# theEricMa/ScaleDreamer

Measured on AMD Instinct MI355X. Metric: ASD train steps/sec (64x64 render, SD2.1), higher is better.
Workload: dtype f32 renderer / f16 diffusion (f32 accumulate); 1 GPU; asd_sd_nerf: 1 view/GPU, 64x64 rays, 512 spp occgrid march, implicit-volume iNGP (16x2 hash grid 2^19, MLP 64), SD-2.1 UNet batch 5 (CFG+Perp-Neg+shifted t), VAE 512^2 fwd+bwd, AdamW; views_per_gpu=1, parallelism=dp1, diffusion_backend=hip, diffusion_weights=seeded random init (seed 1)

## Files before the change

### include/asd_hip.h

```cpp
#ifndef ASD_HIP_H
#define ASD_HIP_H

#include <stdint.h>

#ifdef __cplusplus
extern "C" {
#endif

#define ASD_MAX_LEVELS 16
#define ASD_OK 0
#define ASD_ERR_ARG 1
#define ASD_ERR_LAUNCH 2
#define ASD_ERR_UNSUPPORTED 3

typedef struct asd_grid_meta {
    uint32_t n_levels;
    uint32_t n_features;
    uint32_t n_params;
    uint32_t reserved;
    float    scale[ASD_MAX_LEVELS];
    uint32_t resolution[ASD_MAX_LEVELS];
    uint32_t offset[ASD_MAX_LEVELS];
    uint32_t size[ASD_MAX_LEVELS];
    uint32_t dense[ASD_MAX_LEVELS];
// ... 184 lines not shown
                      float* weights , float* opacity, float* depth, float* rgb_fg ,
                      float* z_var, float* comp_rgb , void* stream);
int asd_composite_bwd(int32_t mode, const float* sigma, const float* t_start, const float* t_end,
                      const float* rgb, const int32_t* offset, const int32_t* count, int32_t n_rays,
                      const float* bg, const float* weights, const float* opacity, const float* depth,
                      const float* d_comp_rgb, const float* d_rgb_fg, const float* d_opacity,
                      const float* d_depth, const float* d_z_var, const float* d_weights,
                      float* d_sigma, float* d_rgb, float* d_bg, void* stream);

typedef struct asd_render_params {
    asd_march_cfg march;
    const asd_grid_meta* meta;
    const asd_field_cfg* field;
    const float* rays_o; const float* rays_d; int32_t n_rays;
    const uint32_t* occ_bits;
    const float* jitter;
    const float* grid; const float* w1d; const float* w2d; const float* w1f; const float* w2f;
    const float* bg;
    float early_stop_eps, alpha_thre;
    int32_t prune;
    int32_t color_act;
    int32_t capacity;
} asd_render_params;
typedef struct asd_render_layout {
    int64_t total_bytes;
    int64_t count, offset, total;
    int64_t c_ray_idx, c_t0, c_t1, c_pts, c_sigma, keep;
    int64_t kept, koff, n_kept;
    int64_t ray_idx , t0, t1, pts, dirs, sigma, feats , enc, weights;
    int64_t opacity, depth, z_var, rgb_fg, comp_rgb;
    int64_t c_feats, c_enc;
} asd_render_layout;
int asd_render_layout_init(int32_t n_rays, int32_t capacity, asd_render_layout* layout);
int asd_render_fwd(const asd_render_params* p, void* workspace, void* stream);
int asd_render_bwd_workspace(const asd_render_params* p, int64_t* n_floats);
int asd_render_bwd(const asd_render_params* p, void* workspace, const float* d_comp_rgb, const float* d_rgb_fg, const float* d_opacity,
                   const float* d_depth, const float* d_z_var, float* d_grid, float* dw1d, float* dw2d, float* dw1f, float* dw2f,
                   float* d_bg, float* bwd_workspace, void* stream);

typedef struct asd_gemm_args {
    const void* A;
    const void* W;
    void*       C;
    int32_t M, N, K;
    int32_t lda, ldw, ldc;
    const void* bias;
    const void* row_bias;
    int32_t rows_per_group;
    const void* residual;
    int32_t ldr;
    int32_t act;
    int32_t out_f32;
    int32_t conv;
    int32_t Hin, Win, Cin, Hout, Wout, stride, pad;
    int32_t upsample;
    const void* zero_page;
    int32_t split_k;
    float*  workspace;
    int32_t tile_cfg;
    int32_t ld_row_bias;
    int32_t group_m, group_n;
    float*  gn_partials;
    int32_t gn_cg;
    int32_t gn_rows;
    const void* gn_bwd_x;
    const float* gn_bwd_fstats;
    const void* gn_bwd_gamma; const void* gn_bwd_beta;
    float   gn_eps;
    int32_t gn_silu;
    int32_t wide_rows;
    int32_t ln_mode;
    float   ln_eps;
    const float* ln_sc;
    float*  ln_stats;
    int32_t a_seg_rows, w_seg_rows;
    int32_t a_seg_off[9], w_seg_off[6];
    int32_t partials_only;
    int32_t gn_apply;
    void*   gn_apply_y;
    const void* gn_apply_gamma; const void* gn_apply_beta;
    float   gn_apply_eps;
    int32_t gn_apply_silu;
    float*  gn_apply_stats;
} asd_gemm_args;
int32_t asd_gemm_gn_records(const asd_gemm_args* args);
int32_t asd_gemm_gn_applies(const asd_gemm_args* args);
int asd_gemm_f16(const asd_gemm_args* args, void* stream);
int asd_gemm_force_tile(int32_t cfg);
enum { ASD_TILE_PLAIN = 0, ASD_TILE_WIN = 1, ASD_TILE_WIN2 = 2, ASD_TILE_PP = 3, ASD_TILE_WS = 4 };
int asd_gemm_tile_info(int32_t i, int32_t* out7);

#define ASD_GN_STATS_FLOATS(batch) (64 * (batch) + 64 * (512 + (batch)))
int asd_groupnorm_f16(const void* x1, int32_t c1, const void* x2, int32_t c2, int32_t batch, int32_t hw,
                      const void* gamma, const void* beta, float eps, int32_t silu, void* y,
                      float* stats ,
                      void* stream);
int asd_groupnorm_ordered_f16(const void* x, int32_t c, int32_t batch, int32_t hw, const void* gamma, const void* beta, float eps,
                              int32_t silu, void* y, float* stats, void* stream);
int asd_groupnorm_apply_f16(const void* x, int32_t c, int32_t batch, int32_t hw, const void* gamma, const void* beta, float eps,
                            int32_t silu, const float* partials, int32_t records, void* y, float* stats, void* stream);
int asd_groupnorm_bwd_f16(const void* x, const void* dy, int32_t c, int32_t batch, int32_t hw, const void* gamma,
                          const void* beta, float eps, int32_t silu, const float* fwd_stats,
                          const void* dx_add ,
                          void* dx, float* bwd_stats , void* stream);
int asd_groupnorm_bwd_apply_f16(const void* x, const void* dy, int32_t c, int32_t batch, int32_t hw, const void* gamma, const void* beta,
                                float eps, int32_t silu, const float* fwd_stats, const float* partials, int32_t records,
                                const void* dx_add, void* dx, float* scratch , void* stream);
int asd_transpose_f16(const void* x, int32_t rows, int32_t cols, int32_t ldx, void* y, int32_t ldy, void* stream);
int asd_layernorm_f16(const void* x, int32_t rows, int32_t c, const void* gamma, const void* beta, float eps,
                      void* y, void* stream);
int asd_softmax_f16(const void* x, int32_t ldx, int32_t rows, int32_t cols, float scale, void* y, int32_t ldy, void* stream);
int asd_softmax_bwd_f16(const void* p, const void* dp, int32_t ld, int32_t rows, int32_t cols, float scale, void* ds,
                        void* stream);
int asd_geglu_f16(const void* h, int32_t rows, int32_t c, void* y, void* stream);
int asd_silu_f16(const void* x, int64_t n, void* y, void* stream);
int asd_timestep_embedding_f16(const float* t, int32_t n, int32_t dim, void* y, void* stream);
int asd_concat_f16(const void* x1, int32_t c1, const void* x2, int32_t c2, int64_t rows, void* y, void* stream);
int asd_attention_f16(const void* q, int32_t ldq, const void* k, int32_t ldk, const void* vT, int32_t ldv,
                      void* o, int32_t ldo, int32_t batch, int32_t heads, int32_t lq, int32_t lk,
                      int32_t lk_stride, float scale, const void* zero_page, void* stream);

int asd_gemm_plan_set(int32_t M, int32_t N, int32_t K, int32_t conv, int32_t s0, int32_t s1, int32_t s2, int32_t s3, int32_t s4,
                      int32_t tile_cfg, int32_t split_k);
int asd_gemm_plan_get(const asd_gemm_args* args, int32_t* tile_cfg, int32_t* split_k);
int asd_gemm_plan_count(void);
uint64_t asd_gemm_plan_generation(void);
int asd_gemm_plan_entry(int32_t i, int32_t* out11 );
int64_t asd_gemm_workspace_bytes(const asd_gemm_args* args);
int asd_gemm_tune(const asd_gemm_args* args, void* scratch, int64_t scratch_bytes, void* stream);
int asd_pad_cast_f16(const float* x, int32_t rows, int32_t c, void* y, int32_t c_pad, void* stream);

typedef struct asd_weight_info { const char* name; int32_t rows, cols; } asd_weight_info;

typedef struct asd_unet_desc {
    int32_t in_channels, out_channels, model_channels, num_res_blocks;
    int32_t n_levels, channel_mult[8];
    int32_t attention_ds_mask;
    int32_t num_head_channels;
    int32_t transformer_depth, context_dim;
    int32_t camera_dim;
} asd_unet_desc;
typedef struct asd_unet asd_unet;
int asd_unet_create(const asd_unet_desc* desc, asd_unet** out);
void asd_unet_destroy(asd_unet* h);
int32_t asd_unet_num_weights(const asd_unet* h);
int asd_unet_weight_info(const asd_unet* h, int32_t i, asd_weight_info* info);
int asd_unet_bind_weights(asd_unet* h, const void* const* device_ptrs, int32_t count);
int64_t asd_unet_workspace_bytes(asd_unet* h, int32_t batch, int32_t H, int32_t W, int32_t n_ctx, int32_t num_frames, int32_t tune);
int asd_unet_fwd(asd_unet* h, const void* x_nhwc, const float* t, const void* context, const void* camera, int32_t batch, int32_t H,
                 int32_t W, int32_t n_ctx, int32_t num_frames, void* workspace, int64_t workspace_bytes, float* eps_nhwc, int32_t tune,
                 void* stream);

int64_t asd_unet_workspace_bytes_shared(asd_unet* h, int32_t batch, int32_t H, int32_t W, int32_t n_ctx, int32_t num_frames, int32_t tune,
                                        int32_t n_uniq);
int asd_unet_fwd_shared(asd_unet* h, const void* x_nhwc, const float* t, const void* context, const void* camera, int32_t batch, int32_t H,
                        int32_t W, int32_t n_ctx, int32_t num_frames, const int32_t* uniq_src_dev, const int32_t* expand_dev, int32_t n_uniq,
                        void* workspace, int64_t workspace_bytes, float* eps_nhwc, int32_t tune, void* stream);
int asd_gather_rows_f16(const void* src, const int32_t* idx_dev, int32_t n_out, int64_t row_halfs, void* dst, void* stream);

typedef struct asd_vae_desc {
    int32_t in_channels, ch, n_levels, ch_mult[8], num_res_blocks, z_channels, embed_dim;
} asd_vae_desc;
typedef struct asd_vae_enc asd_vae_enc;
int asd_vae_enc_create(const asd_vae_desc* desc, asd_vae_enc** out);
void asd_vae_enc_destroy(asd_vae_enc* h);
int32_t asd_vae_enc_num_weights(const asd_vae_enc* h);
int asd_vae_enc_weight_info(const asd_vae_enc* h, int32_t i, asd_weight_info* info);
int asd_vae_enc_bind_weights(asd_vae_enc* h, const void* const* device_ptrs, int32_t count);
int64_t asd_vae_enc_workspace_bytes(asd_vae_enc* h, int32_t batch, int32_t H, int32_t W, int32_t tune);
int asd_vae_enc_fwd(asd_vae_enc* h, const void* x_nhwc32, int32_t batch, int32_t H, int32_t W, void* workspace, int64_t workspace_bytes,
                    float* moments_nhwc, int32_t tune, void* stream);
int asd_vae_enc_bwd(asd_vae_enc* h, const float* d_moments_nhwc, int32_t batch, int32_t H, int32_t W, void* workspace,
                    int64_t workspace_bytes, void* dx_nhwc32, int32_t tune, void* stream);

typedef struct asd_vae_dec asd_vae_dec;
int asd_vae_dec_create(const asd_vae_desc* desc, asd_vae_dec** out);
void asd_vae_dec_destroy(asd_vae_dec* h);
int32_t asd_vae_dec_num_weights(const asd_vae_dec* h);
int asd_vae_dec_weight_info(const asd_vae_dec* h, int32_t i, asd_weight_info* info);
int asd_vae_dec_bind_weights(asd_vae_dec* h, const void* const* device_ptrs, int32_t count);
int64_t asd_vae_dec_workspace_bytes(asd_vae_dec* h, int32_t batch, int32_t hl, int32_t wl, int32_t tune);
int asd_vae_dec_fwd(asd_vae_dec* h, const void* z_nhwc32, int32_t batch, int32_t hl, int32_t wl, void* workspace, int64_t workspace_bytes,
                    void* x_nhwc32, int32_t tune, void* stream);

int asd_image_prep_fwd(const float* rgb, int32_t B, int32_t h, int32_t w, int32_t H, int32_t W, void* x_nhwc32, void* stream);
int asd_image_prep_bwd(const void* dx_nhwc32, int32_t B, int32_t h, int32_t w, int32_t H, int32_t W, float* d_rgb, void* stream);
int asd_latents_fwd(const float* moments_nhwc, const float* post_noise, const float* noise, const int64_t* t, const int64_t* t_plus,
                    const float* alphas_cumprod, int32_t B, int32_t C, int32_t hl, int32_t wl, float scaling, int32_t n_rep,
                    float* latents, void* unet_x, float* unet_t, void* stream);
int asd_score_fwd(const float* eps_nhwc, int32_t B, int32_t C, int32_t hw, int32_t n_neg, const float* neg_w, float guidance_scale,
                  const int64_t* t, const float* alphas_cumprod, int32_t weighting, float grad_clip, float* grad, float* sumsq,
                  float* loss_and_norm, void* stream);
int asd_prompt_context(const float* text_vd, const float* uncond_vd, int32_t n_dir, int32_t n_tok, int32_t dim, const float* elevation,
                       const float* azimuth, int32_t batch, int32_t layout, const float* params15, float neg_scale, void* context_f16,
                       int32_t ctx_stride, float* neg_w, void* stream);
int asd_latents_bwd(const float* grad, const float* moments_nhwc, const float* post_noise, const float* upstream, int32_t B, int32_t C,
                    int32_t hl, int32_t wl, float scaling, float* d_moments_nhwc, void* stream);
int asd_latent_input_fwd(const float* render_bhwc, const float* noise, const int64_t* t, const int64_t* t_plus, const float* alphas_cumprod,
                         int32_t B, int32_t h, int32_t w, int32_t hl, int32_t wl, int32_t n_rep, float* latents, void* unet_x, float* unet_t,
                         void* stream);
int asd_latent_input_bwd(const float* grad, const float* upstream, int32_t B, int32_t h, int32_t w, int32_t hl, int32_t wl, float* d_render_bhwc,
                         void* stream);
int asd_latent_decode_prep(const float* latents_bhwc, int32_t B, int32_t h, int32_t w, int32_t hl, int32_t wl, float inv_scaling,
// ... 175 lines not shown
```

### scaledreamer_amd/_lib.py

```python
from __future__ import annotations

import ctypes as C
import os
from typing import Optional

import torch

_HERE = os.path.dirname(os.path.abspath(__file__))
LIB_PATH = os.environ.get("ASD_HIP_LIB") or os.path.join(_HERE, "libasd_hip.so")
ASD_MAX_LEVELS = 16

ASD_BIAS_CONST, ASD_BIAS_BLOB_MAGIC3D, ASD_BIAS_BLOB_DREAMFUSION, ASD_BIAS_SPHERE = 0, 1, 2, 3
ASD_FIELD_DENSITY, ASD_FIELD_SDF = 0, 1
ASD_ACT_SOFTPLUS, ASD_ACT_EXP, ASD_ACT_TRUNC_EXP, ASD_ACT_NONE = 0, 1, 2, 3


class AsdError(RuntimeError):
    pass


class GridMeta(C.Structure):
    _fields_ = [
        ("n_levels", C.c_uint32),
        ("n_features", C.c_uint32),
        ("n_params", C.c_uint32),
        ("reserved", C.c_uint32),
        ("scale", C.c_float * ASD_MAX_LEVELS),
        ("resolution", C.c_uint32 * ASD_MAX_LEVELS),
        ("offset", C.c_uint32 * ASD_MAX_LEVELS),
        ("size", C.c_uint32 * ASD_MAX_LEVELS),
        ("dense", C.c_uint32 * ASD_MAX_LEVELS),
    ]


class FieldCfg(C.Structure):
    _fields_ = [
        ("bbox_min", C.c_float * 3),
        ("bbox_max", C.c_float * 3),
        ("radius", C.c_float),
        ("bias_mode", C.c_int32),
        ("bias_value", C.c_float),
        ("blob_scale", C.c_float),
        ("blob_std", C.c_float),
        ("activation", C.c_int32),
        ("fd_eps", C.c_float),
        ("n_hidden", C.c_int32),
        ("n_feature_dims", C.c_int32),
        ("field_mode", C.c_int32),
    ]


class MarchCfg(C.Structure):
    _fields_ = [
        ("aabb", C.c_float * 6),
        ("resolution", C.c_int32),
        ("near_plane", C.c_float),
        ("far_plane", C.c_float),
        ("step", C.c_float),
        ("max_steps", C.c_int32),
    ]


class GemmArgs(C.Structure):
    _fields_ = [
        ("A", C.c_void_p), ("W", C.c_void_p), ("C", C.c_void_p),
        ("M", C.c_int32), ("N", C.c_int32), ("K", C.c_int32),
        ("lda", C.c_int32), ("ldw", C.c_int32), ("ldc", C.c_int32),
        ("bias", C.c_void_p), ("row_bias", C.c_void_p), ("rows_per_group", C.c_int32),
        ("residual", C.c_void_p), ("ldr", C.c_int32), ("act", C.c_int32), ("out_f32", C.c_int32),
        ("conv", C.c_int32), ("Hin", C.c_int32), ("Win", C.c_int32), ("Cin", C.c_int32), ("Hout", C.c_int32),
        ("Wout", C.c_int32), ("stride", C.c_int32), ("pad", C.c_int32), ("upsample", C.c_int32),
        ("zero_page", C.c_void_p), ("split_k", C.c_int32), ("workspace", C.c_void_p),
        ("tile_cfg", C.c_int32), ("ld_row_bias", C.c_int32), ("group_m", C.c_int32), ("group_n", C.c_int32),
        ("gn_partials", C.c_void_p), ("gn_cg", C.c_int32), ("gn_rows", C.c_int32),
        ("gn_bwd_x", C.c_void_p), ("gn_bwd_fstats", C.c_void_p), ("gn_bwd_gamma", C.c_void_p), ("gn_bwd_beta", C.c_void_p),
        ("gn_eps", C.c_float), ("gn_silu", C.c_int32), ("wide_rows", C.c_int32),
        ("ln_mode", C.c_int32), ("ln_eps", C.c_float), ("ln_sc", C.c_void_p), ("ln_stats", C.c_void_p),
        ("a_seg_rows", C.c_int32), ("w_seg_rows", C.c_int32), ("a_seg_off", C.c_int32 * 9), ("w_seg_off", C.c_int32 * 6),
        ("partials_only", C.c_int32),
        ("gn_apply", C.c_int32), ("gn_apply_y", C.c_void_p), ("gn_apply_gamma", C.c_void_p), ("gn_apply_beta", C.c_void_p),
        ("gn_apply_eps", C.c_float), ("gn_apply_silu", C.c_int32), ("gn_apply_stats", C.c_void_p),
    ]


class RenderParams(C.Structure):
    _fields_ = [("march", MarchCfg), ("meta", C.c_void_p), ("field", C.c_void_p), ("rays_o", C.c_void_p), ("rays_d", C.c_void_p), ("n_rays", C.c_int32),
                ("occ_bits", C.c_void_p), ("jitter", C.c_void_p), ("grid", C.c_void_p), ("w1d", C.c_void_p), ("w2d", C.c_void_p), ("w1f", C.c_void_p),
                ("w2f", C.c_void_p), ("bg", C.c_void_p), ("early_stop_eps", C.c_float), ("alpha_thre", C.c_float), ("prune", C.c_int32),
                ("color_act", C.c_int32), ("capacity", C.c_int32)]


RENDER_LAYOUT_FIELDS = ["total_bytes", "count", "offset", "total", "c_ray_idx", "c_t0", "c_t1", "c_pts", "c_sigma", "keep", "kept", "koff", "n_kept",
                        "ray_idx", "t0", "t1", "pts", "dirs", "sigma", "feats", "enc", "weights", "opacity", "depth", "z_var", "rgb_fg", "comp_rgb",
                        "c_feats", "c_enc"]


class RenderLayout(C.Structure):
    _fields_ = [(k, C.c_int64) for k in RENDER_LAYOUT_FIELDS]


class Conv3dDesc(C.Structure):
    _fields_ = [("N", C.c_int32), ("D", C.c_int32), ("H", C.c_int32), ("W", C.c_int32), ("Cin", C.c_int32), ("Cout", C.c_int32),
                ("amax_x", C.c_void_p), ("amax_dy", C.c_void_p)]


class Conv3dEpilogue(C.Structure):
    _fields_ = [("bias", C.c_void_p), ("noise", C.c_void_p), ("noise_strength", C.c_void_p), ("act", C.c_int32), ("gain", C.c_float),
                ("clamp", C.c_float), ("amax_out", C.c_void_p)]


class OptTensor(C.Structure):
    _fields_ = [("p", C.c_void_p), ("g", C.c_void_p), ("m", C.c_void_p), ("v", C.c_void_p), ("n2", C.c_void_p), ("prev", C.c_void_p),
                ("n", C.c_int64), ("lr", C.c_float), ("weight_decay", C.c_float), ("bias_correction1", C.c_float),
                ("bias_correction2", C.c_float), ("bias_correction2_sqrt", C.c_float)]


class TritxDesc(C.Structure):
    _fields_ = [("n_layers", C.c_int32), ("dim", C.c_int32), ("heads", C.c_int32), ("cond_dim", C.c_int32), ("cond_tokens", C.c_int32),
                ("hidden", C.c_int32), ("low_res", C.c_int32), ("out_channels", C.c_int32), ("eps", C.c_float), ("grads_prezeroed", C.c_int32)]


class WeightInfo(C.Structure):
    _fields_ = [("name", C.c_char_p), ("rows", C.c_int32), ("cols", C.c_int32)]


class UNetDesc(C.Structure):
    _fields_ = [("in_channels", C.c_int32), ("out_channels", C.c_int32), ("model_channels", C.c_int32), ("num_res_blocks", C.c_int32),
                ("n_levels", C.c_int32), ("channel_mult", C.c_int32 * 8), ("attention_ds_mask", C.c_int32),
                ("num_head_channels", C.c_int32), ("transformer_depth", C.c_int32), ("context_dim", C.c_int32), ("camera_dim", C.c_int32)]


class VaeDesc(C.Structure):
    _fields_ = [("in_channels", C.c_int32), ("ch", C.c_int32), ("n_levels", C.c_int32), ("ch_mult", C.c_int32 * 8),
                ("num_res_blocks", C.c_int32), ("z_channels", C.c_int32), ("embed_dim", C.c_int32)]


class MtLayout(C.Structure):
    _fields_ = [(k, C.c_int64) for k in ("n_edge_slots", "n_tet_slots", "edge_off", "tet_off", "scan", "counts", "total")]


class AtlasLayout(C.Structure):
    _fields_ = [(k, C.c_int32) for k in ("n_faces", "texture_size", "gutter", "n", "c", "L")]


class ImagePanel(C.Structure):
    _fields_ = [("src", C.c_void_p), ("minmax", C.c_void_p), ("kind", C.c_int32), ("normalize", C.c_int32), ("lo", C.c_float), ("hi", C.c_float)]


ASD_PANEL_RGB, ASD_PANEL_GRAYSCALE = 0, 1

_lib: Optional[C.CDLL] = None

SYMBOLS = [
    "asd_grid_meta_init", "asd_hashgrid_fwd", "asd_hashgrid_bwd",
    "asd_field_density", "asd_field_fwd", "asd_field_bwd_workspace", "asd_field_bwd",
    "asd_field_analytic_fwd", "asd_field_analytic_bwd_workspace", "asd_field_analytic_bwd",
    "asd_envmap_fwd", "asd_envmap_bwd",
    "asd_importance_resample", "asd_transmittance_cdf", "asd_merge_sorted", "asd_voxel_sample_fwd", "asd_voxel_sample_bwd", "asd_voxel_sample_bwd_rows",
    "asd_triplane_sample_fwd", "asd_triplane_sample_bwd", "asd_triplane_sample_bwd_rows", "asd_relayout_f32",
    "asd_volsdf_edges", "asd_volsdf_samples", "asd_volsdf_proposal_cdf", "asd_volsdf_composite_fwd", "asd_volsdf_composite_bwd",
    "asd_neus_step_alpha", "asd_neus_prune_count", "asd_neus_composite_fwd", "asd_neus_composite_bwd",
    "asd_generate_rays", "asd_march_count", "asd_scan_i32", "asd_march_write", "asd_prune_count", "asd_compact",
    "asd_occgrid_update", "asd_composite_fwd", "asd_composite_bwd",
    "asd_gemm_f16", "asd_gemm_force_tile", "asd_groupnorm_f16", "asd_groupnorm_bwd_f16", "asd_transpose_f16", "asd_layernorm_f16", "asd_softmax_f16", "asd_softmax_bwd_f16", "asd_geglu_f16", "asd_silu_f16",
    "asd_timestep_embedding_f16", "asd_concat_f16", "asd_attention_f16",
    "asd_gemm_plan_set", "asd_gemm_plan_get", "asd_gemm_plan_count", "asd_gemm_plan_generation", "asd_gemm_plan_entry", "asd_gemm_tile_info", "asd_gemm_workspace_bytes", "asd_gemm_tune", "asd_gemm_gn_records", "asd_gemm_gn_applies", "asd_groupnorm_apply_f16", "asd_groupnorm_bwd_apply_f16", "asd_groupnorm_ordered_f16",
    "asd_pad_cast_f16",
    "asd_image_prep_fwd", "asd_image_prep_bwd", "asd_latents_fwd", "asd_score_fwd", "asd_latents_bwd", "asd_prompt_context",
    "asd_unet_create", "asd_unet_destroy", "asd_unet_num_weights", "asd_unet_weight_info", "asd_unet_bind_weights",
    "asd_unet_workspace_bytes", "asd_unet_fwd", "asd_unet_workspace_bytes_shared", "asd_unet_fwd_shared", "asd_gather_rows_f16",
    "asd_vae_enc_create", "asd_vae_enc_destroy", "asd_vae_enc_num_weights", "asd_vae_enc_weight_info", "asd_vae_enc_bind_weights",
    "asd_vae_enc_workspace_bytes", "asd_vae_enc_fwd", "asd_vae_enc_bwd",
    "asd_vae_dec_create", "asd_vae_dec_destroy", "asd_vae_dec_num_weights", "asd_vae_dec_weight_info", "asd_vae_dec_bind_weights",
    "asd_vae_dec_workspace_bytes", "asd_vae_dec_fwd",
    "asd_latent_input_fwd", "asd_latent_input_bwd", "asd_latent_decode_prep", "asd_image_from_decoder",
    "asd_adamw_f32", "asd_adan_f32",
    "asd_conv3d_workspace_bytes", "asd_conv3d_fwd", "asd_conv3d_dgrad", "asd_conv3d_wgrad", "asd_layer_act_bwd", "asd_upsample3d_fwd", "asd_upsample3d_bwd",
    "asd_torgb_fwd", "asd_torgb_bwd", "asd_absmax_f32", "asd_voxfield_fwd", "asd_voxfield_bwd_workspace", "asd_voxfield_bwd",
    "asd_trifield_fwd_workspace", "asd_trifield_fwd", "asd_trifield_bwd_workspace", "asd_trifield_bwd",
    "asd_render_layout_init", "asd_render_fwd", "asd_render_bwd_workspace", "asd_render_bwd",
    "asd_tx_pack_weight", "asd_tx_linear_workspace", "asd_tx_linear", "asd_tx_wgrad_workspace", "asd_tx_linear_wgrad", "asd_tx_layernorm_fwd", "asd_tx_layernorm_bwd",
    "asd_tx_attention_workspace", "asd_tx_attention_fwd", "asd_tx_attention_bwd",
    "asd_tritx_packed_floats", "asd_tritx_save_floats", "asd_tritx_workspace_floats", "asd_tritx_pack", "asd_tritx_fwd", "asd_tritx_bwd",
    "asd_mt_workspace", "asd_mt_count", "asd_mt_emit", "asd_mt_case_table", "asd_scan_i32_blocks_workspace", "asd_scan_i32_blocks",
    "asd_mesh_cc_round", "asd_mesh_face_counts", "asd_mesh_keep", "asd_mesh_compact",
    "asd_atlas_layout", "asd_atlas_uv", "asd_atlas_bake", "asd_atlas_pack_u8",
    "asd_image_minmax_workspace", "asd_image_minmax_f32", "asd_image_grid_u8",
    "asd_clip_preprocess_u8", "asd_clip_embed_f16", "asd_quick_gelu_f16", "asd_clip_score_workspace", "asd_clip_score_f32",
    "asd_text_embed_f16", "asd_attention_causal_f16", "asd_gelu_f16",
    "asd_comm_unique_id", "asd_comm_create", "asd_comm_destroy", "asd_allreduce_mean_f32",
    "asd_version", "asd_last_error", "asd_modulated_weights_fwd", "asd_modulated_weights_bwd", "asd_timestep_plus", "asd_loss_tail_fwd", "asd_loss_tail_bwd", "asd_probe_events", "asd_probe_mark",
]


def lib() -> C.CDLL:
    global _lib
    if _lib is None:
        if not os.path.exists(LIB_PATH):
            raise AsdError(
                f"{LIB_PATH} not found: build it with `python -c 'import __graft_entry__ as g; g.build()'` "
                "(make -C scaledreamer_amd/csrc). The HIP path has no fallback."
            )
        l = C.CDLL(LIB_PATH)
        l.asd_last_error.restype = C.c_char_p
        l.asd_version.restype = C.c_char_p
        l.asd_grid_meta_init.restype = C.c_uint32
        l.asd_grid_meta_init.argtypes = [C.POINTER(GridMeta), C.c_uint32, C.c_uint32, C.c_uint32, C.c_uint32, C.c_double]
        for fn in ("asd_gemm_workspace_bytes", "asd_unet_workspace_bytes", "asd_unet_workspace_bytes_shared", "asd_vae_enc_workspace_bytes",
                   "asd_vae_dec_workspace_bytes",
                   "asd_conv3d_workspace_bytes", "asd_tx_linear_workspace", "asd_tx_wgrad_workspace", "asd_tx_attention_workspace",
                   "asd_tritx_packed_floats", "asd_tritx_save_floats", "asd_tritx_workspace_floats", "asd_image_minmax_workspace",
                   "asd_clip_score_workspace"):
            getattr(l, fn).restype = C.c_int64
        l.asd_unet_destroy.restype = None
        l.asd_vae_enc_destroy.restype = None
        l.asd_unet_destroy.argtypes = [C.c_void_p]
        l.asd_vae_enc_destroy.argtypes = [C.c_void_p]
        l.asd_vae_dec_destroy.restype = None
        l.asd_vae_dec_destroy.argtypes = [C.c_void_p]
        vp, i, f = C.c_void_p, C.c_int32, C.c_float
        l.asd_neus_step_alpha.argtypes = [vp, i, vp, vp, f, i, vp, vp]
        l.asd_neus_prune_count.argtypes = [vp, vp, vp, i, vp, f, i, f, f, vp, vp, vp]
        l.asd_neus_composite_fwd.argtypes = [vp] * 6 + [i, vp, f, i, vp, vp, vp, i] + [vp] * 7
        l.asd_neus_composite_bwd.argtypes = [vp] * 6 + [i, vp, f, i, vp, vp, vp, i] + [vp] * 14
        l.asd_latent_input_fwd.argtypes = [vp] * 5 + [i] * 6 + [vp] * 4
        l.asd_latent_input_bwd.argtypes = [vp, vp] + [i] * 5 + [vp, vp]
        l.asd_latent_decode_prep.argtypes = [vp] + [i] * 5 + [f, vp, vp, vp]
        l.asd_image_from_decoder.argtypes = [vp, C.c_int64, vp, vp, vp]
        l.asd_vae_dec_workspace_bytes.argtypes = [vp, i, i, i, i]
        l.asd_groupnorm_ordered_f16.argtypes = [vp, i, i, i, vp, vp, f, i, vp, vp, vp]
        l.asd_vae_dec_fwd.argtypes = [vp, vp, i, i, i, vp, C.c_int64, vp, i, vp]
        _lib = l
    return _lib


def check(status: int) -> None:
    if status != 0:
        raise AsdError(f"libasd_hip error {status}: {lib().asd_last_error().decode()}")


def ptr(t: Optional[torch.Tensor]):
    if t is None:
        return C.c_void_p(0)
    if not t.is_contiguous():
        raise AsdError("non-contiguous tensor passed to the C ABI")
    return C.c_void_p(t.data_ptr())


# ... 21 lines not shown
```

### scaledreamer_amd/csrc/attention.hip

```cpp
#include "asd_common.h"

typedef _Float16 half_t;
typedef half_t half8 __attribute__((ext_vector_type(8)));
typedef half_t half4 __attribute__((ext_vector_type(4)));
typedef float floatx4 __attribute__((ext_vector_type(4)));
#define GLOBAL_AS __attribute__((address_space(1)))
#define LDS_AS __attribute__((address_space(3)))

typedef float float2_ __attribute__((ext_vector_type(2)));

__device__ __forceinline__ float max3f(float a, float b, float c) {
    float r;
    asm("v_max3_f32 %0, %1, %2, %3" : "=v"(r) : "v"(a), "v"(b), "v"(c));
    return r;
}
__device__ __forceinline__ float fma1(float a, float b, float c) {
    float r;
    asm("v_fma_f32 %0, %1, %2, %3" : "=v"(r) : "v"(a), "v"(b), "v"(c));
    return r;
}
__device__ __forceinline__ float rows_max(float v) {
    auto t = __builtin_amdgcn_permlane16_swap(__float_as_uint(v), __float_as_uint(v), false, false);
    v = max3f(__uint_as_float(t[0]), __uint_as_float(t[1]), -3.0e38f);
    t = __builtin_amdgcn_permlane32_swap(__float_as_uint(v), __float_as_uint(v), false, false);
    return max3f(__uint_as_float(t[0]), __uint_as_float(t[1]), -3.0e38f);
}

#define HD 64
#define ATTN_DEFER_LOG2 8.0f
#define KT 64

struct AttnArgs {
    const half_t* q; int ldq;
    const half_t* k; int ldk;
    const half_t* vT; int ldv;
    half_t* o; int ldo;
    int batch, heads, lq, lk, lk_stride;
    float scale;
    const char* zero;
};

template <int QS>
__global__ __launch_bounds__(256, QS == 2 ? 4 : 2) void attention_fwd_kernel(const AttnArgs p) {
    constexpr int QW = 16 * QS, QB = 4 * QW;
    extern __shared__ __attribute__((aligned(16))) char smem[];
    constexpr int TILE_BYTES = KT * HD * 2;
    const int tid = threadIdx.x, lane = tid & 63, wave = tid >> 6;
    const int qblocks = (p.lq + QB - 1) / QB, items = qblocks * p.heads * p.batch;
    const int per = (items + 7) >> 3, item = ((int)blockIdx.x & 7) * per + ((int)blockIdx.x >> 3);
    if (((int)blockIdx.x >> 3) >= per || item >= items) return;
    const int b = item / (qblocks * p.heads), h = (item / qblocks) % p.heads;
    const int q0 = (item % qblocks) * QB + wave * QW;
    const int lq16 = lane & 15, lg = lane >> 4;

    half8 qf[QS][2];
#pragma unroll
    for (int qs = 0; qs < QS; ++qs) {
        int qi = q0 + qs * 16 + lq16;
        if (qi >= p.lq) qi = p.lq - 1;
        const half_t* src = p.q + ((size_t)b * p.lq + qi) * p.ldq + h * HD;
#pragma unroll
        for (int ks = 0; ks < 2; ++ks) qf[qs][ks] = *(const half8*)(src + ks * 32 + lg * 8);
    }

    const int srow = lane >> 3, pch = lane & 7;
    const size_t kbase = (size_t)b * p.lk_stride;
    auto issue = [&](int t, int buf) {
        char* Ks = smem + buf * 2 * TILE_BYTES;
        char* Vs = Ks + TILE_BYTES;
        const int key0 = t * KT;
#pragma unroll
        for (int i = 0; i < 2; ++i) {
            const int row = (wave * 2 + i) * 8 + srow;
            {
                const int c = pch ^ (row & 7);
                const int key = key0 + row;
                const char* src = key < p.lk_stride ? (const char*)(p.k + (kbase + key) * p.ldk + h * HD) + c * 16 : p.zero;
                __builtin_amdgcn_global_load_lds((const GLOBAL_AS void*)src, (LDS_AS void*)(Ks + (wave * 2 + i) * 8 * 128), 16, 0, 0);
            }
            {
                const int c = pch ^ ((row >> 1) & 7);
                const char* src = key0 + c * 8 < p.lk_stride
                                      ? (const char*)(p.vT + (size_t)(h * HD + row) * p.ldv + kbase + key0) + c * 16 : p.zero;
                __builtin_amdgcn_global_load_lds((const GLOBAL_AS void*)src, (LDS_AS void*)(Vs + (wave * 2 + i) * 8 * 128), 16, 0, 0);
            }
        }
    };

    floatx4 oacc[QS][4];
#pragma unroll
    for (int qs = 0; qs < QS; ++qs)
#pragma unroll
        for (int dt = 0; dt < 4; ++dt) oacc[qs][dt] = floatx4{0.f, 0.f, 0.f, 0.f};
    float m_run[QS];
#pragma unroll
    for (int qs = 0; qs < QS; ++qs) m_run[qs] = -1e30f;
    floatx4 lacc[QS];
#pragma unroll
    for (int qs = 0; qs < QS; ++qs) lacc[qs] = floatx4{0.f, 0.f, 0.f, 0.f};
    const half_t one_or_zero = lq16 == 0 ? (half_t)1.f : (half_t)0.f;
    const half8 ones_row0 = {one_or_zero, one_or_zero, one_or_zero, one_or_zero, one_or_zero, one_or_zero, one_or_zero, one_or_zero};

    const int n_tiles = (p.lk + KT - 1) / KT;
    const float sl2 = p.scale * 1.44269504088896340736f;
    issue(0, 0);
    __builtin_amdgcn_s_waitcnt(0);
    __syncthreads();
    for (int t = 0; t < n_tiles; ++t) {
        const int buf = t & 1;
        if (t + 1 < n_tiles) issue(t + 1, buf ^ 1);
        const char* Ks = smem + buf * 2 * TILE_BYTES;
        const char* Vs = Ks + TILE_BYTES;

        floatx4 s[4][QS];
#pragma unroll
        for (int kt = 0; kt < 4; ++kt) {
            const int row = kt * 16 + lq16;
            half8 kf[2];
#pragma unroll
            for (int ks = 0; ks < 2; ++ks) kf[ks] = *(const half8*)(Ks + row * 128 + (((ks * 4 + lg) ^ (row & 7)) * 16));
#pragma unroll
            for (int qs = 0; qs < QS; ++qs) {
                floatx4 a = {0.f, 0.f, 0.f, 0.f};
                a = __builtin_amdgcn_mfma_f32_16x16x32_f16(kf[0], qf[qs][0], a, 0, 0, 0);
                a = __builtin_amdgcn_mfma_f32_16x16x32_f16(kf[1], qf[qs][1], a, 0, 0, 0);
                s[kt][qs] = a;
            }
        }
        const int key_base = t * KT + lg * 4;
        half8 pb[2][QS];
        if (t == n_tiles - 1 && (p.lk & (KT - 1)) != 0) {
            asm volatile("" ::: "memory");
#pragma unroll
            for (int qs = 0; qs < QS; ++qs)
#pragma unroll
                for (int kt = 0; kt < 4; ++kt)
#pragma unroll
                    for (int r = 0; r < 4; ++r)
                        if (key_base + kt * 16 + r >= p.lk) s[kt][qs][r] = -1e30f;
        }
#pragma unroll
        for (int qs = 0; qs < QS; ++qs) {
            const float a0 = max3f(s[0][qs][0], s[0][qs][1], s[0][qs][2]), a1 = max3f(s[0][qs][3], s[1][qs][0], s[1][qs][1]);
            const float a2 = max3f(s[1][qs][2], s[1][qs][3], s[2][qs][0]), a3 = max3f(s[2][qs][1], s[2][qs][2], s[2][qs][3]);
            const float a4 = max3f(s[3][qs][0], s[3][qs][1], s[3][qs][2]);
            float mx = max3f(max3f(a0, a1, a2), max3f(a3, a4, s[3][qs][3]), -3.0e38f);
            mx = rows_max(mx);
            const float cand = mx * sl2;
            const bool grow = __builtin_amdgcn_ballot_w64(cand > m_run[qs] + ATTN_DEFER_LOG2) != 0;
            const float m_new = grow ? max3f(m_run[qs], cand, -3.0e38f) : m_run[qs];
            const float alpha = grow ? __builtin_amdgcn_exp2f(m_run[qs] - m_new) : 1.f;
            const float2_ sl2v = {sl2, sl2}, nm = {-m_new, -m_new};
#pragma unroll
            for (int kt = 0; kt < 4; ++kt) {
                float2_ x01, x23;
                if constexpr (QS == 4) {
                    x01 = float2_{fma1(s[kt][qs][0], sl2, -m_new), fma1(s[kt][qs][1], sl2, -m_new)};
                    x23 = float2_{fma1(s[kt][qs][2], sl2, -m_new), fma1(s[kt][qs][3], sl2, -m_new)};
                } else {
                    x01 = __builtin_elementwise_fma(__builtin_shufflevector(s[kt][qs], s[kt][qs], 0, 1), sl2v, nm);
                    x23 = __builtin_elementwise_fma(__builtin_shufflevector(s[kt][qs], s[kt][qs], 2, 3), sl2v, nm);
                }
                const float2_ e01 = {__builtin_amdgcn_exp2f(x01[0]), __builtin_amdgcn_exp2f(x01[1])};
                const float2_ e23 = {__builtin_amdgcn_exp2f(x23[0]), __builtin_amdgcn_exp2f(x23[1])};
                half8& dst = pb[kt >> 1][qs];
                dst[(kt & 1) * 4 + 0] = (half_t)e01[0]; dst[(kt & 1) * 4 + 1] = (half_t)e01[1];
                dst[(kt & 1) * 4 + 2] = (half_t)e23[0]; dst[(kt & 1) * 4 + 3] = (half_t)e23[1];
            }
            if (grow) {
#pragma unroll
                for (int dt = 0; dt < 4; ++dt) {
                    oacc[qs][dt][0] *= alpha; oacc[qs][dt][1] *= alpha; oacc[qs][dt][2] *= alpha; oacc[qs][dt][3] *= alpha;
                }
                lacc[qs][0] *= alpha;
            }
            m_run[qs] = m_new;
        }
#pragma unroll
        for (int j = 0; j < 2; ++j) {
#pragma unroll
            for (int dt = 0; dt < 4; ++dt) {
                const int row = dt * 16 + lq16;
                const int sw = (row >> 1) & 7;
                const int c_lo = (4 * j + (lg >> 1)) ^ sw, c_hi = (4 * j + 2 + (lg >> 1)) ^ sw;
                const half4 v_lo = *(const volatile LDS_AS half4*)(Vs + row * 128 + c_lo * 16 + (lg & 1) * 8);
                const half4 v_hi = *(const volatile LDS_AS half4*)(Vs + row * 128 + c_hi * 16 + (lg & 1) * 8);
                const half8 vf = half8{v_lo[0], v_lo[1], v_lo[2], v_lo[3], v_hi[0], v_hi[1], v_hi[2], v_hi[3]};
#pragma unroll
                for (int qs = 0; qs < QS; ++qs) oacc[qs][dt] = __builtin_amdgcn_mfma_f32_16x16x32_f16(vf, pb[j][qs], oacc[qs][dt], 0, 0, 0);
            }
#pragma unroll
            for (int qs = 0; qs < QS; ++qs) lacc[qs] = __builtin_amdgcn_mfma_f32_16x16x32_f16(ones_row0, pb[j][qs], lacc[qs], 0, 0, 0);
        }
        __syncthreads();
    }

#pragma unroll
    for (int qs = 0; qs < QS; ++qs) {
        const int qi = q0 + qs * 16 + lq16;
        const float inv = 1.f / __shfl(lacc[qs][0], lq16, 64);
        if (qi >= p.lq) continue;
        half_t* dst = p.o + ((size_t)b * p.lq + qi) * p.ldo + h * HD;
#pragma unroll
        for (int dt = 0; dt < 4; ++dt) {
            const floatx4 v = oacc[qs][dt];
            const half4 o = {(half_t)(v[0] * inv), (half_t)(v[1] * inv), (half_t)(v[2] * inv), (half_t)(v[3] * inv)};
            *(half4*)(dst + dt * 16 + lg * 4) = o;
        }
    }
}

extern "C" {

int asd_attention_f16(const void* q, int32_t ldq, const void* k, int32_t ldk, const void* vT, int32_t ldv, void* o,
                      int32_t ldo, int32_t batch, int32_t heads, int32_t lq, int32_t lk, int32_t lk_stride, float scale,
                      const void* zero_page, void* stream) {
    ASD_CHECK_ARG(q && k && vT && o && zero_page, "null argument");
    ASD_CHECK_ARG(batch > 0 && heads > 0 && lq > 0 && lk > 0 && lk_stride >= lk, "bad sizes");
    ASD_CHECK_ARG(ldq % 8 == 0 && ldk % 8 == 0 && ldv % 8 == 0 && ldo % 4 == 0 && lk_stride % 8 == 0,
                  "leading dimensions / key stride must keep 16-byte alignment");
    AttnArgs a{(const half_t*)q, ldq, (const half_t*)k, ldk, (const half_t*)vT, ldv, (half_t*)o, ldo,
               batch, heads, lq, lk, lk_stride, scale, (const char*)zero_page};
    const bool wide = lk >= 2048 && lq >= 2048;
    if (wide) {
        const dim3 grid(8 * asd_div_up(asd_div_up(lq, 256) * heads * batch, 8));
        hipLaunchKernelGGL(attention_fwd_kernel<4>, grid, dim3(256), 4 * KT * HD * 2, (hipStream_t)stream, a);
    } else {
        const dim3 grid(8 * asd_div_up(asd_div_up(lq, 128) * heads * batch, 8));
        hipLaunchKernelGGL(attention_fwd_kernel<2>, grid, dim3(256), 4 * KT * HD * 2, (hipStream_t)stream, a);
    }
    ASD_LAUNCH_CHECK();
    return ASD_OK;
}

}
```

### scaledreamer_amd/csrc/gemm.hip

```cpp
#include <stdlib.h>

#include "asd_common.h"
#include <map>
#include <atomic>
#include <mutex>
#include <cstring>
#include <iterator>

#include "gemm_tile.h"


template <int BM, int BN, int WM, int WN, bool CONV, int NST = 2, int KG = 1, bool LN = false>
__global__ __launch_bounds__(WM * WN * KG * 64) void gemm_f16_kernel(const asd_gemm_args p) {
    constexpr int NW = WM * WN;
    constexpr int TM = BM / WM / 16, TN = BN / WN / 16;
    constexpr int RB = 128;
    constexpr int A_BYTES = BM * RB, B_BYTES = BN * RB;
    constexpr int STAGE_BYTES = A_BYTES + B_BYTES;
    constexpr int ASLABS = BM / 8, TSLABS = (BM + BN) / 8;
    constexpr int SPW = (TSLABS + NW - 1) / NW;
    static_assert(BM % (WM * 16) == 0 && BN % (WN * 16) == 0, "wave tile must be a multiple of 16 x 16");
    static_assert(NST == 2 || TSLABS % NW == 0, "ring variants count their loads per wave: every wave must own the same number of slabs");
    static_assert(KG == 1 || NST == 2, "k-groups use the two-stage loop");
    extern __shared__ __attribute__((aligned(16))) char smem[];

    const int tid = threadIdx.x, lane = tid & 63;
    const int wave_all = __builtin_amdgcn_readfirstlane(tid >> 6);
    const int kg = KG > 1 ? wave_all / NW : 0;
    const int wave = wave_all - kg * NW;
    char* const gsm = smem + kg * (NST * STAGE_BYTES);
    const int wm = wave / WN, wn = wave % WN;
    const bool up3 = CONV && p.upsample == 3;
    const int up_mq = up3 ? p.M >> 2 : 1;
    const int tiles_pp = (up_mq + BM - 1) / BM;
    const int tiles_m = up3 ? 4 * tiles_pp : (p.M + BM - 1) / BM, tiles_n = (p.N + BN - 1) / BN;
    int item, tm_, tn_;
    if (!asd_xcd_item(blockIdx.x, tiles_m * tiles_n * p.split_k, item)) return;
    const int kz = item / (tiles_m * tiles_n);
    asd_grouped_tile(item - kz * tiles_m * tiles_n, tiles_m, tiles_n, p.group_m, p.group_n, tm_, tn_);
    const int parity = up3 ? tm_ / tiles_pp : 0;
    const int m0 = up3 ? parity * up_mq + (tm_ - parity * tiles_pp) * BM : tm_ * BM, n0 = tn_ * BN;
    const int m_lim = up3 ? (parity + 1) * up_mq : p.M;
    const int k_steps_total = (p.K + 63) / 64;
    const int k_per = (k_steps_total + p.split_k - 1) / p.split_k;
    const int ks0 = kz * k_per, ks1 = min(k_steps_total, ks0 + k_per);

    const int lrow = lane >> 3, pchunk = lane & 7;
    const char* zero = (const char*)p.zero_page;
    const bool fast_conv = CONV && (p.upsample == 0 || p.upsample == 3) && (p.Cin & 63) == 0;
    const int par_a = parity >> 1, par_b = parity & 1;
    const char* const Wp = (const char*)p.W + ((CONV && p.upsample == 3) ? (size_t)parity * p.N * p.ldw * 2 : 0);
    const int lch = pchunk ^ lrow;
    constexpr int ASPW = (ASLABS + NW - 1) / NW;
    const char* a0 = nullptr;
    const char* c_base[CONV ? ASPW : 1];
    int c_yx[CONV ? ASPW : 1];
    if (!CONV) {
        a0 = (const char*)p.A + (size_t)(m0 + lrow) * p.lda * 2 + lch * 16;
    } else {
#pragma unroll
        for (int j = 0; j < ASPW; ++j) {
            const int slab = wave + j * NW;
            int m = min(m0 + slab * 8 + lrow, m_lim - 1);
            int hw = p.Hout * p.Wout, wrow = p.Wout;
            if (p.upsample == 3) { m -= parity * up_mq; hw = p.Hin * p.Win; wrow = p.Win; }
            const int b = m / hw, r = m - b * hw;
            int y = r / wrow, x = r - y * wrow;
            c_base[j] = (const char*)p.A + (size_t)b * p.Hin * p.Win * p.Cin * 2;
            if (fast_conv) {
                y *= p.stride; x *= p.stride;
                c_base[j] += ((size_t)(y * p.Win + x) * p.Cin) * 2 + lch * 16;
            }
            c_yx[j] = (y << 16) | x;
        }
    }
    constexpr bool WIDE_OK = (BN / WN) % 32 == 0;
    const bool wide = WIDE_OK && p.wide_rows;
    const int wl = wide ? wide_lane_row(lrow) : lrow;
    auto w_slab_rows = [&](int ws) { return wide ? wide_slab_rows(ws) : ws * 8; };
    const char* w0 = Wp + (size_t)(n0 + wl) * p.ldw * 2 + lch * 16;
    const size_t a_slab_stride = (size_t)8 * p.lda * 2, w_row_stride = (size_t)p.ldw * 2;
    unsigned roff[SPW];
#pragma unroll
    for (int j = 0; j < SPW; ++j) {
        const int slab = wave + j * NW;
        if (slab >= ASLABS) {
            const int row = min(n0 + w_slab_rows(slab - ASLABS) + wl, p.N - 1);
            roff[j] = (unsigned)row * (unsigned)(p.ldw * 2) + lch * 16 + (ks0 + kg) * 128;
            if (!CONV && p.w_seg_rows > 0) {
                const int seg = row / p.w_seg_rows;
                roff[j] = (unsigned)(row - seg * p.w_seg_rows) * (unsigned)(p.ldw * 2) + (unsigned)p.w_seg_off[seg] + lch * 16 + (ks0 + kg) * 128;
            }
        } else {
            const int row = min(m0 + slab * 8 + lrow, p.M - 1);
            roff[j] = CONV ? 0u : (unsigned)row * (unsigned)(p.lda * 2) + lch * 16 + (ks0 + kg) * 128;
// ... 209 lines not shown
        }
    } else {
    int k = ks0;
    while (k < ks1 && !live(k)) ++k;
    if (k < ks1) {
        issue(k, 0);
        for (int stage = 0;; stage ^= 1) {
            asm volatile("s_waitcnt vmcnt(0)" ::: "memory");
            __builtin_amdgcn_s_barrier();
            int kn = k + 1;
            while (kn < ks1 && !live(kn)) ++kn;
            if (kn < ks1) issue(kn, stage ^ 1);
            compute(gsm + stage * STAGE_BYTES);
            if (kn >= ks1) break;
            k = kn;
        }
    }
    }
    if constexpr (KG == 1) ln_extract();

    const int em = lane & 15, en = (lane >> 4) * 4;
    auto out_row = [&](int i) {
        const int m = m0 + wm * (BM / WM) + i * 16 + em;
        if (m >= m_lim) return -1;
        if (CONV && p.upsample == 3) {
            const int q = m - parity * up_mq, hwq = p.Hin * p.Win;
            const int bb = q / hwq, r = q - bb * hwq, y = r / p.Win, x = r - y * p.Win;
            return (bb * p.Hout + 2 * y + par_a) * p.Wout + 2 * x + par_b;
        }
        return m;
    };
    if (KG > 1 && kg != 0) {
        if (p.split_k == 1 && p.act != 2 && p.gn_partials != nullptr) {
            __syncthreads(); __syncthreads();
            __syncthreads();
        }
        return;
    }
    if (p.split_k > 1) {
        tile_epilogue<TM, TN>(p, acc, n0 + wn * (BN / WN), kz, m0, out_row, false, nullptr);
        return;
    }
    float ln_mean[LN ? TM : 1], ln_rstd[LN ? TM : 1];
    if constexpr (LN) {
        const float inv_k = 1.f / (float)p.K;
#pragma unroll
        for (int i = 0; i < TM; ++i) {
            ln_mean[i] = ls1[i] * inv_k;
            ln_rstd[i] = rsqrtf(fmaxf(ls2[i] * inv_k - ln_mean[i] * ln_mean[i], 0.f) + p.ln_eps);
            const int m = m0 + wm * (BM / WM) + i * 16 + em;
            if (p.ln_stats && n0 == 0 && wn == 0 && lane < 16 && m < p.M) { p.ln_stats[2 * m] = ln_mean[i]; p.ln_stats[2 * m + 1] = ln_rstd[i]; }
        }
    }
    if (p.act == 2) {
        if constexpr (TN % 2 == 0) {
#pragma unroll
            for (int i = 0; i < TM; ++i) {
                const int m = m0 + wm * (BM / WM) + i * 16 + em;
                if (m >= p.M) continue;
#pragma unroll
                for (int j = 0; j < TN; j += 2) {
                    const int n = n0 + wn * (BN / WN) + j * 16 + en;
                    if (n + 16 >= p.N) continue;
                    const half4 bx = *(const half4*)((const half_t*)p.bias + n), bg = *(const half4*)((const half_t*)p.bias + n + 16);
                    float va[4] = {acc[i][j][0], acc[i][j][1], acc[i][j][2], acc[i][j][3]};
                    float vg[4] = {acc[i][j + 1][0], acc[i][j + 1][1], acc[i][j + 1][2], acc[i][j + 1][3]};
                    if (p.ln_mode) {
                        ln_fold<4>(p, va, m, n, LN ? ln_mean[i] : 0.f, LN ? ln_rstd[i] : 0.f);
                        ln_fold<4>(p, vg, m, n + 16, LN ? ln_mean[i] : 0.f, LN ? ln_rstd[i] : 0.f);
                    }
                    half4 o;
#pragma unroll
                    for (int r = 0; r < 4; ++r)
                        o[r] = (half_t)((va[r] + (float)bx[r]) * gelu_erf(vg[r] + (float)bg[r]));
                    *(half4*)((half_t*)p.C + (size_t)m * p.ldc + (n >> 5) * 16 + (n & 15)) = o;
                }
            }
        }
        return;
    }
    const bool gn = p.gn_partials != nullptr;
    float* gn_lds = (float*)smem;
    if (gn) gn_tile_begin(gn_lds);
    tile_epilogue<TM, TN>(p, acc, n0 + wn * (BN / WN), kz, m0, out_row, gn, gn_lds, LN ? ln_mean : nullptr, LN ? ln_rstd : nullptr);
    if (gn) gn_tile_end(p, gn_lds, (m0 / BM) * ((p.N + BN - 1) / BN) + n0 / BN);
}

#define LDS_READ16(dst, addr, OFF) asm volatile("ds_read_b128 %0, %1 offset:%2" : "=&v"(dst) : "v"(addr), "n"(OFF) : "memory")
#define LGKM_WAIT(N, F)                                                                                                  \
    asm volatile("s_waitcnt lgkmcnt(" #N ")"                                                                             \
                 : "+v"(F.a[0]), "+v"(F.a[1]), "+v"(F.a[2]), "+v"(F.a[3]), "+v"(F.w[0]), "+v"(F.w[1]), "+v"(F.w[2]), "+v"(F.w[3]))

template <int BN>
__global__ __launch_bounds__(512) void conv3x3_win_kernel(const asd_gemm_args p) {
    constexpr int WN = 2, TM = 4, TN = BN / WN / 16;
    constexpr int RB = 128;
    constexpr int WIN = 18, WIN_ROWS = WIN * WIN, WIN_SLABS = (WIN_ROWS + 7) / 8;
    constexpr int A_BYTES = WIN_SLABS * 8 * RB, W_BYTES = BN * RB;
    constexpr int WSLABS = BN / 8, WSPW = (WSLABS + 7) / 8;
    extern __shared__ __attribute__((aligned(16))) char smem[];
    char* const a_buf = smem;
    char* const w_buf = smem + 2 * A_BYTES;

    const int tid = threadIdx.x, lane = tid & 63, wave = tid >> 6;
    const int wm = wave >> 1, wn = wave & 1;
    const int tiles_x = p.Wout / 16, tiles_y = p.Hout / 16;
    const int tiles_m = (p.M / (p.Hout * p.Wout)) * tiles_y * tiles_x;
    const int tiles_n = (p.N + BN - 1) / BN;
    int item, tm, tn_;
    if (!asd_xcd_item(blockIdx.x, tiles_m * tiles_n * p.split_k, item)) return;
    const int kz = item / (tiles_m * tiles_n);
    asd_grouped_tile(item - kz * tiles_m * tiles_n, tiles_m, tiles_n, p.group_m, p.group_n, tm, tn_);
    const int n0 = tn_ * BN;
    const int b = tm / (tiles_y * tiles_x), tr = tm - b * tiles_y * tiles_x;
    const int y0 = (tr / tiles_x) * 16, x0 = (tr - (tr / tiles_x) * tiles_x) * 16;
    const int n_chunks = p.Cin / 64;
    const int c_per = (n_chunks + p.split_k - 1) / p.split_k;
    const int c0 = kz * c_per, c1 = min(n_chunks, c0 + c_per);
    const int steps = (c1 - c0) * 9;

    const int lrow = lane >> 3, pchunk = lane & 7;
    const char* zero = (const char*)p.zero_page;
    const char* img = (const char*)p.A + (size_t)b * p.Hin * p.Win * p.Cin * 2;
    const bool wide = p.wide_rows != 0;
    const int wl = wide ? wide_lane_row(lrow) : lrow;
    const char* w0 = (const char*)p.W + (size_t)(n0 + wl) * p.ldw * 2 + (pchunk ^ lrow) * 16;
    const size_t w_row_stride = (size_t)p.ldw * 2;

    auto load_window_slab = [&](int slab, int chunk, char* dst_buf) {
        const int wrow = slab * 8 + lrow;
        const int wy = (wrow * 3641) >> 16, wx = wrow - wy * WIN;
        const int yi = y0 - 1 + wy, xi = x0 - 1 + wx;
        const bool ok = wrow < WIN_ROWS && (unsigned)yi < (unsigned)p.Hin && (unsigned)xi < (unsigned)p.Win;
        const char* src = ok ? img + ((size_t)(yi * p.Win + xi) * p.Cin + chunk * 64) * 2 + (pchunk ^ (wx & 7)) * 16 : zero;
        load_slab(src, dst_buf + slab * 8 * RB);
    };
    auto load_w_tile = [&](int step, char* dst_buf) {
        const int chunk = c0 + step / 9, tap = step - (step / 9) * 9;
        const size_t koff = ((size_t)tap * p.Cin + chunk * 64) * 2;
#pragma unroll
        for (int j = 0; j < WSPW; ++j) {
            const int slab = wave + j * 8;
            if (slab >= WSLABS) continue;
            const int wr = wide ? wide_slab_rows(slab) : slab * 8;
            const char* src = (n0 + wr + wl < p.N) ? w0 + wr * w_row_stride + koff : zero;
            load_slab(src, dst_buf + slab * 8 * RB);
        }
    };

    floatx4 acc[TM][TN];
#pragma unroll
    for (int i = 0; i < TM; ++i)
#pragma unroll
        for (int j = 0; j < TN; ++j) acc[i][j] = floatx4{0.f, 0.f, 0.f, 0.f};

    const int frow = lane & 15, fq = lane >> 4;
    const unsigned lds_a = (unsigned)(size_t)a_buf + (unsigned)((wm * 4 * WIN + frow) * RB);
    const unsigned lds_w = (unsigned)(size_t)w_buf + (unsigned)((wn * (BN / WN) + frow) * RB);
    const unsigned fsww[2] = {(unsigned)(((fq) ^ (frow & 7)) * 16), (unsigned)(((4 + fq) ^ (frow & 7)) * 16)};
    struct Frag { half8 a[4], w[4]; };
    static_assert(TM == 4 && (TN == 4 || TN == 2), "fragment sets are written for 4 x {2, 4} sub-tiles");

    auto read_frags = [&](Frag& f, int s, int kh) {
        const int cl = s / 9, tap = s - cl * 9;
        const int ky = tap / 3, kx = tap - ky * 3;
        const unsigned aa = lds_a + (unsigned)((cl & 1) * A_BYTES + (ky * WIN + kx) * RB) + (unsigned)(((kh * 4 + fq) ^ ((frow + kx) & 7)) * 16);
        const unsigned wa = lds_w + (unsigned)((s & 3) * W_BYTES) + fsww[kh];
// ... 139 lines not shown
    const int fb0 = (wn * (BN / WN) + frow) * RB;
    const int fswb[2] = {((fq) ^ (frow & 7)) * 16, ((4 + fq) ^ (frow & 7)) * 16};

    if (steps > 0) {
        for (int slab = wave; slab < WIN_SLABS; slab += NW) load_window_slab(slab, c0, a_buf);
        load_w_tile(0, w_buf);
#pragma unroll 1
        for (int s = 0; s < steps; ++s) {
            const int cl = s / 9, tap = s - cl * 9;
            if (tap == 0 && s > 0) {
                __builtin_amdgcn_s_barrier();
                for (int slab = wave; slab < WIN_SLABS; slab += NW) load_window_slab(slab, c0 + cl, a_buf);
            }
            asm volatile("s_waitcnt vmcnt(0)" ::: "memory");
            __builtin_amdgcn_s_barrier();
            if (s + 1 < steps) load_w_tile(s + 1, w_buf + ((s + 1) & 1) * W_BYTES);
            const char* Wt = w_buf + (s & 1) * W_BYTES;
            const int ky = tap / 3, kx = tap - ky * 3;
            const char* Ar = a_buf + ((wm * 4 + ky) * WIN + frow + kx) * RB;
            const int csw = (frow + kx) & 7;
            if constexpr (NW == 4) {
                half8 xa[2][TM], wb[2][TN];
#pragma unroll
                for (int kh = 0; kh < 2; ++kh) {
                    const char* Ak = Ar + (((kh * 4 + fq) ^ csw) * 16);
#pragma unroll
                    for (int i = 0; i < TM; ++i) xa[kh][i] = *(const half8*)(Ak + i * WIN * RB);
#pragma unroll
                    for (int j = 0; j < TN; ++j) wb[kh][j] = *(const half8*)(Wt + fb0 + fswb[kh] + j * 16 * RB);
                }
                __builtin_amdgcn_sched_barrier(0);
#pragma unroll
                for (int kh = 0; kh < 2; ++kh)
#pragma unroll
                    for (int i = 0; i < TM; ++i)
#pragma unroll
                        for (int j = 0; j < TN; ++j)
                            acc[i][j] = __builtin_amdgcn_mfma_f32_16x16x32_f16(wb[kh][j], xa[kh][i], acc[i][j], 0, 0, 0);
            } else {
#pragma unroll
            for (int kh = 0; kh < 2; ++kh) {
                half8 xa[TM], wb[TN];
                const char* Ak = Ar + (((kh * 4 + fq) ^ csw) * 16);
#pragma unroll
                for (int i = 0; i < TM; ++i) xa[i] = *(const half8*)(Ak + i * WIN * RB);
#pragma unroll
                for (int j = 0; j < TN; ++j) wb[j] = *(const half8*)(Wt + fb0 + fswb[kh] + j * 16 * RB);
#pragma unroll
                for (int i = 0; i < TM; ++i)
#pragma unroll
                    for (int j = 0; j < TN; ++j)
                        acc[i][j] = __builtin_amdgcn_mfma_f32_16x16x32_f16(wb[j], xa[i], acc[i][j], 0, 0, 0);
            }
            }
        }
    }

    const bool gn = p.gn_partials != nullptr && p.split_k == 1;
    float* gn_lds = (float*)smem;
    if (gn) gn_tile_begin(gn_lds);
    tile_epilogue<TM, TN>(p, acc, n0 + wn * (BN / WN), kz, b * p.Hout * p.Wout,
                          [&](int i) { return (b * p.Hout + y0 + wm * 4 + i) * p.Wout + x0 + frow; }, gn, gn_lds);
    if (gn) gn_tile_end(p, gn_lds, tm * tiles_n + tn_);
}

__global__ __launch_bounds__(256) void splitk_epilogue_kernel(const asd_gemm_args p, int splits) {
    const size_t q = (size_t)blockIdx.x * 256 + threadIdx.x;
    const size_t total4 = (size_t)p.M * p.N / 4;
    if (q >= total4) return;
    const int m = (int)((q * 4) / p.N), n = (int)((q * 4) % p.N);
    floatx4 v = {0.f, 0.f, 0.f, 0.f};
    for (int s = 0; s < splits; ++s) {
        const floatx4 t = *(const floatx4*)(p.workspace + ((size_t)s * p.M + m) * p.N + n);
        v[0] += t[0]; v[1] += t[1]; v[2] += t[2]; v[3] += t[3];
    }
    if (p.bias) {
        const half4 b = *(const half4*)((const half_t*)p.bias + n);
        v[0] += (float)b[0]; v[1] += (float)b[1]; v[2] += (float)b[2]; v[3] += (float)b[3];
    }
    if (p.row_bias) {
        const half4 b = *(const half4*)((const half_t*)p.row_bias + (size_t)(m / p.rows_per_group) * p.ld_row_bias + n);
        v[0] += (float)b[0]; v[1] += (float)b[1]; v[2] += (float)b[2]; v[3] += (float)b[3];
    }
    if (p.act == 1) {
#pragma unroll
        for (int r = 0; r < 4; ++r) v[r] = asd_silu_fast(v[r]);
    }
    if (p.residual) {
        const half4 b = *(const half4*)((const half_t*)p.residual + (size_t)m * p.ldr + n);
        v[0] += (float)b[0]; v[1] += (float)b[1]; v[2] += (float)b[2]; v[3] += (float)b[3];
    }
    if (p.out_f32) {
        *(floatx4*)((float*)p.C + (size_t)m * p.ldc + n) = v;
    } else {
        half4 o = {(half_t)v[0], (half_t)v[1], (half_t)v[2], (half_t)v[3]};
        *(half4*)((half_t*)p.C + (size_t)m * p.ldc + n) = o;
    }
}

__global__ __launch_bounds__(256) void splitk_epilogue_gn_kernel(const asd_gemm_args p, int splits) {
    __shared__ float lds64[64];
    const int tiles_n = p.N / 64;
    const int mb = blockIdx.x / tiles_n, nb = blockIdx.x - mb * tiles_n;
    const int tx = threadIdx.x & 15, ty = threadIdx.x >> 4;
    const int n = nb * 64 + tx * 4;
    if (threadIdx.x < 64) lds64[threadIdx.x] = 0.f;
    __syncthreads();
    floatx4 cs = {0.f, 0.f, 0.f, 0.f}, cq = {0.f, 0.f, 0.f, 0.f};
    half4 bias = {0, 0, 0, 0};
    if (p.bias) bias = *(const half4*)((const half_t*)p.bias + n);
    floatx4 v[4];
    int mrow[4];
#pragma unroll
    for (int i = 0; i < 4; ++i) {
        v[i] = floatx4{0.f, 0.f, 0.f, 0.f};
        mrow[i] = min(mb * 64 + i * 16 + ty, p.M - 1);
    }
    for (int s = 0; s < splits; ++s) {
        floatx4 t[4];
#pragma unroll
        for (int i = 0; i < 4; ++i) t[i] = *(const floatx4*)(p.workspace + ((size_t)s * p.M + mrow[i]) * p.N + n);
#pragma unroll
        for (int i = 0; i < 4; ++i) { v[i][0] += t[i][0]; v[i][1] += t[i][1]; v[i][2] += t[i][2]; v[i][3] += t[i][3]; }
    }
#pragma unroll
    for (int i = 0; i < 4; ++i) {
        const int m = mb * 64 + i * 16 + ty;
        if (m >= p.M) continue;
        floatx4 w = v[i];
        w[0] += (float)bias[0]; w[1] += (float)bias[1]; w[2] += (float)bias[2]; w[3] += (float)bias[3];
        if (p.row_bias) {
            const half4 b = *(const half4*)((const half_t*)p.row_bias + (size_t)(m / p.rows_per_group) * p.ld_row_bias + n);
            w[0] += (float)b[0]; w[1] += (float)b[1]; w[2] += (float)b[2]; w[3] += (float)b[3];
        }
        if (p.act == 1) {
#pragma unroll
            for (int r = 0; r < 4; ++r) w[r] = asd_silu_fast(w[r]);
        }
        if (p.residual) {
            const half4 b = *(const half4*)((const half_t*)p.residual + (size_t)m * p.ldr + n);
            w[0] += (float)b[0]; w[1] += (float)b[1]; w[2] += (float)b[2]; w[3] += (float)b[3];
        }
        const half4 o = {(half_t)w[0], (half_t)w[1], (half_t)w[2], (half_t)w[3]};
        *(half4*)((half_t*)p.C + (size_t)m * p.ldc + n) = o;
#pragma unroll
        for (int r = 0; r < 4; ++r) { const float f = (float)o[r]; cs[r] += f; cq[r] = fmaf(f, f, cq[r]); }
    }
#pragma unroll
    for (int r = 0; r < 4; ++r) {
        const int g = (n + r) / p.gn_cg;
        atomicAdd(&lds64[2 * g], cs[r]);
        atomicAdd(&lds64[2 * g + 1], cq[r]);
    }
    __syncthreads();
    if (threadIdx.x < 64) p.gn_partials[(size_t)blockIdx.x * 64 + threadIdx.x] = lds64[threadIdx.x];
}

#define GNA_THREADS 1024
template <int NV>
__global__ __launch_bounds__(GNA_THREADS) void splitk_epilogue_gnapply_kernel(const asd_gemm_args p, int splits, float inv_cnt ) {
    __shared__ float red[2 * (GNA_THREADS / 64)];
    const int cg = p.gn_cg, g4 = cg >> 2, rows = p.gn_rows;
    const int b = blockIdx.x >> 5, g = blockIdx.x & 31;
    const int n0 = g * cg, total = rows * g4, tid = threadIdx.x;
    floatx4 v[NV];
    int mrow[NV], ncol[NV];
// ... 51 lines not shown
        if (live) *(half4*)((half_t*)p.C + (size_t)m * p.ldc + n) = o;
#pragma unroll
        for (int r = 0; r < 4; ++r) {
            const float f = (float)o[r];
            v[i][r] = f;
            if (live) { cs += f; cq = fmaf(f, f, cq); }
        }
    }
#pragma unroll
    for (int off = 32; off > 0; off >>= 1) { cs += __shfl_xor(cs, off, 64); cq += __shfl_xor(cq, off, 64); }
    if ((tid & 63) == 0) { red[(tid >> 6) * 2] = cs; red[(tid >> 6) * 2 + 1] = cq; }
    __syncthreads();
    float sum = 0.f, sq = 0.f;
#pragma unroll
    for (int w = 0; w < GNA_THREADS / 64; ++w) { sum += red[2 * w]; sq += red[2 * w + 1]; }
    if (p.gn_apply_stats && tid == 0) { p.gn_apply_stats[b * 64 + g * 2] = sum; p.gn_apply_stats[b * 64 + g * 2 + 1] = sq; }
    const float mean = sum * inv_cnt;
    const float var = fmaxf(sq * inv_cnt - mean * mean, 0.f);
    const float rstd = rsqrtf(var + p.gn_apply_eps);
#pragma unroll
    for (int i = 0; i < NV; ++i) {
        if (tid + GNA_THREADS * i >= total) continue;
        const int m = mrow[i], n = ncol[i];
        const half4 gm = *(const half4*)((const half_t*)p.gn_apply_gamma + n), bt = *(const half4*)((const half_t*)p.gn_apply_beta + n);
        half4 o;
#pragma unroll
        for (int r = 0; r < 4; ++r) {
            const float sa = rstd * (float)gm[r];
            float f = fmaf(v[i][r], sa, (float)bt[r] - mean * sa);
            if (p.gn_apply_silu) f = asd_silu_fast(f);
            o[r] = (half_t)f;
        }
        *(half4*)((half_t*)p.gn_apply_y + (size_t)m * p.N + n) = o;
    }
}

static int asd_gemm_gn_apply_nv(const asd_gemm_args* a) {
    if (!a->gn_apply || a->split_k <= 1 || a->partials_only || a->out_f32 || a->act == 2 || a->gn_bwd_x) return 0;
    if (a->gn_cg < 4 || a->gn_cg % 4 || a->N != 32 * a->gn_cg || a->gn_rows < 1 || a->M % a->gn_rows || a->ldc % 4) return 0;
    if (a->conv && a->upsample == 3) return 0;
    const int need = (a->gn_rows * (a->gn_cg / 4) + GNA_THREADS - 1) / GNA_THREADS;
    return need <= 1 ? 1 : need <= 3 ? 3 : 0;
}

static void asd_launch_splitk_epilogue(const asd_gemm_args* a, hipStream_t s) {
    const int nv = a->gn_apply_y ? asd_gemm_gn_apply_nv(a) : 0;
    if (nv > 0) {
        const dim3 grid((a->M / a->gn_rows) * 32);
        const float inv_cnt = 1.f / ((float)a->gn_rows * (float)a->gn_cg);
        if (nv == 1) hipLaunchKernelGGL(splitk_epilogue_gnapply_kernel<1>, grid, dim3(GNA_THREADS), 0, s, *a, a->split_k, inv_cnt);
        else hipLaunchKernelGGL(splitk_epilogue_gnapply_kernel<3>, grid, dim3(GNA_THREADS), 0, s, *a, a->split_k, inv_cnt);
        return;
    }
    const size_t total4 = (size_t)a->M * a->N / 4;
    if (a->gn_partials) hipLaunchKernelGGL(splitk_epilogue_gn_kernel, dim3((a->M / 64) * (a->N / 64)), dim3(256), 0, s, *a, a->split_k);
    else hipLaunchKernelGGL(splitk_epilogue_kernel, dim3(asd_div_up(total4, 256)), dim3(256), 0, s, *a, a->split_k);
}


struct asd_gemm_tile {
    int kind;
    int bm, bn, wm, wn;
    int nst, kg;
    int (*launch)(asd_gemm_args* a, hipStream_t s);
};

static void asd_pick_group(int tiles_m, int tiles_n, int bm, int bn, size_t lds, int* gm, int* gn) {
    const int conc = 32 * (2 * lds <= 160 * 1024 ? 2 : 1);
    int m = (int)lroundf(sqrtf((float)conc * (float)bn / (float)bm));
    m = m < 1 ? 1 : (m > tiles_m ? tiles_m : m);
    int n = conc / m;
    n = n < 1 ? 1 : (n > tiles_n ? tiles_n : n);
    if (n == tiles_n) { m = conc / n; m = m < 1 ? 1 : (m > tiles_m ? tiles_m : m); }
    *gm = m; *gn = n;
}

template <int BM, int BN, int WM, int WN, int NST, int KG>
static int asd_launch_plain(asd_gemm_args* a, hipStream_t s) {
    const int tiles = (a->conv && a->upsample == 3 ? 4 * asd_div_up(a->M / 4, BM) : asd_div_up(a->M, BM)) * asd_div_up(a->N, BN);
    const size_t lds = (size_t)NST * KG * (BM + BN) * 128;
    if (a->group_m < 1 || a->group_n < 1) asd_pick_group(asd_div_up(a->M, BM), asd_div_up(a->N, BN), BM, BN, lds, &a->group_m, &a->group_n);
    const dim3 grid(8 * asd_div_up(tiles * a->split_k, 8)), block(WM * WN * KG * 64);
    if (a->conv) asd_launch_lds<gemm_f16_kernel<BM, BN, WM, WN, true, NST, KG, false>>(grid, block, lds, s, *a);
    else if (a->ln_mode == 1) asd_launch_lds<gemm_f16_kernel<BM, BN, WM, WN, false, NST, KG, true>>(grid, block, lds, s, *a);
    else asd_launch_lds<gemm_f16_kernel<BM, BN, WM, WN, false, NST, KG, false>>(grid, block, lds, s, *a);
    return ASD_OK;
}

template <bool TWO, int BN, int NW>
static int asd_launch_window(asd_gemm_args* a, hipStream_t s) {
    const size_t lds = (size_t)(TWO ? 1 : 2) * (41 * 1024 + 2 * BN * 128);
    const int tiles_n = asd_div_up(a->N, BN);
    if (a->group_m < 1 || a->group_n < 1) asd_pick_group(a->M / 256, tiles_n, 256, BN, TWO ? (size_t)80 * 1024 : lds, &a->group_m, &a->group_n);
    const dim3 grid(8 * asd_div_up((a->M / 256) * tiles_n * a->split_k, 8)), block(NW * 64);
    if constexpr (TWO) asd_launch_lds<conv3x3_win2_kernel<BN, NW>>(grid, block, lds, s, *a);
    else asd_launch_lds<conv3x3_win_kernel<BN>>(grid, block, lds, s, *a);
    return ASD_OK;
}

size_t asd_conv_pp_lds_bytes(int tm, int tn);
template <int TM, int TN> void asd_conv_pp_launch(const asd_gemm_args* a, int blocks, hipStream_t s);
template <int TM, int TN>
static int asd_launch_pp(asd_gemm_args* a, hipStream_t s) {
    const int tiles_m = a->M / (64 * TM), tiles_n = a->N / (32 * TN);
    if (a->group_m < 1 || a->group_n < 1) asd_pick_group(tiles_m, tiles_n, 64 * TM, 32 * TN, asd_conv_pp_lds_bytes(TM, TN), &a->group_m, &a->group_n);
    asd_conv_pp_launch<TM, TN>(a, 8 * asd_div_up(tiles_m * tiles_n * a->split_k, 8), s);
    return ASD_OK;
}

int asd_conv_ws_launch(const asd_gemm_args* a, hipStream_t s);
static int asd_launch_ws(asd_gemm_args* a, hipStream_t s) {
    if (asd_conv_ws_launch(a, s) != ASD_OK) { asd_set_error("weight-streaming convolution: bad image count"); return ASD_ERR_ARG; }
    return ASD_OK;
}

template <int KIND, int BM, int BN, int WM, int WN, int NST, int KG>
static int asd_tile_launch(asd_gemm_args* a, hipStream_t s) {
    if constexpr (KIND == ASD_TILE_PLAIN) return asd_launch_plain<BM, BN, WM, WN, NST, KG>(a, s);
    else {
        static_assert(NST == 2 && KG == 1, "only the plain kernel has a ring depth and k-groups to choose");
        if constexpr (KIND == ASD_TILE_WIN) { static_assert(BM == 256 && WM * WN == 8, "window: 256 pixels, eight waves"); return asd_launch_window<false, BN, 8>(a, s); }
        else if constexpr (KIND == ASD_TILE_WIN2) { static_assert(BM == 256, "window: 256 pixels"); return asd_launch_window<true, BN, WM * WN>(a, s); }
        else if constexpr (KIND == ASD_TILE_PP) { static_assert(BM % 64 == 0 && BN % 32 == 0 && WM * WN == 8, "ping-pong: eight waves"); return asd_launch_pp<BM / 64, BN / 32>(a, s); }
        else { static_assert(KIND == ASD_TILE_WS && BM == 320 && BN == 64 && WM * WN == 4, "weight streaming: 5 x 64 rows, four waves"); return asd_launch_ws(a, s); }
    }
}
#define ASD_TILE(KIND, BM, BN, WM, WN, NST, KG) {ASD_TILE_##KIND, BM, BN, WM, WN, NST, KG, &asd_tile_launch<ASD_TILE_##KIND, BM, BN, WM, WN, NST, KG>}
static constexpr asd_gemm_tile asd_gemm_tiles[] = {
    ASD_TILE(PLAIN, 128, 64, 2, 2, 2, 1), ASD_TILE(PLAIN, 128, 128, 2, 2, 2, 1), ASD_TILE(PLAIN, 256, 64, 4, 2, 2, 1), ASD_TILE(PLAIN, 256, 128, 4, 2, 2, 1),
    ASD_TILE(PLAIN, 128, 320, 2, 4, 2, 1), ASD_TILE(PLAIN, 256, 256, 2, 4, 2, 1), ASD_TILE(PLAIN, 256, 320, 2, 4, 2, 1), ASD_TILE(PLAIN, 320, 128, 5, 2, 2, 1),
    ASD_TILE(WIN, 256, 64, 4, 2, 2, 1), ASD_TILE(WIN, 256, 128, 4, 2, 2, 1), ASD_TILE(WIN2, 256, 64, 4, 2, 2, 1), ASD_TILE(WIN2, 256, 128, 4, 2, 2, 1),
    ASD_TILE(PLAIN, 64, 64, 2, 2, 2, 1),
    ASD_TILE(WIN2, 256, 64, 4, 1, 2, 1), ASD_TILE(WIN2, 256, 128, 4, 1, 2, 1),
    ASD_TILE(PLAIN, 64, 64, 2, 2, 4, 1), ASD_TILE(PLAIN, 64, 64, 2, 2, 2, 2), ASD_TILE(PLAIN, 64, 64, 2, 2, 2, 4), ASD_TILE(PLAIN, 128, 64, 2, 2, 2, 2),
    ASD_TILE(PLAIN, 128, 128, 2, 2, 2, 2),
    ASD_TILE(PP, 512, 128, 4, 2, 2, 1), ASD_TILE(PP, 256, 256, 4, 2, 2, 1), ASD_TILE(PP, 256, 320, 4, 2, 2, 1), ASD_TILE(PP, 256, 128, 4, 2, 2, 1),
    ASD_TILE(PP, 256, 160, 4, 2, 2, 1),
    ASD_TILE(WS, 320, 64, 2, 2, 2, 1),
    ASD_TILE(PLAIN, 128, 64, 2, 2, 6, 1), ASD_TILE(PLAIN, 64, 64, 2, 2, 8, 1), ASD_TILE(PLAIN, 128, 128, 2, 2, 4, 1)};
#define ASD_GEMM_NCFG ((int)(sizeof(asd_gemm_tiles) / sizeof(asd_gemm_tiles[0])))

static constexpr bool asd_cfg_is(int cfg, int kind, int bm, int bn) {
    return asd_gemm_tiles[cfg].kind == kind && asd_gemm_tiles[cfg].bm == bm && asd_gemm_tiles[cfg].bn == bn;
}
static_assert(asd_cfg_is(ASD_CFG_128x64, ASD_TILE_PLAIN, 128, 64) && asd_cfg_is(ASD_CFG_128x128, ASD_TILE_PLAIN, 128, 128) &&
              asd_cfg_is(ASD_CFG_256x64, ASD_TILE_PLAIN, 256, 64) && asd_cfg_is(ASD_CFG_256x128, ASD_TILE_PLAIN, 256, 128) &&
              asd_cfg_is(ASD_CFG_256x256, ASD_TILE_PLAIN, 256, 256) && asd_cfg_is(ASD_CFG_320x128, ASD_TILE_PLAIN, 320, 128) &&
              asd_cfg_is(ASD_CFG_WIN_64, ASD_TILE_WIN, 256, 64) && asd_cfg_is(ASD_CFG_WIN_128, ASD_TILE_WIN, 256, 128) &&
              asd_cfg_is(ASD_CFG_WIN2_64, ASD_TILE_WIN2, 256, 64) && asd_cfg_is(ASD_CFG_WIN2_128, ASD_TILE_WIN2, 256, 128),
              "a named tile configuration moved");

static bool asd_cfg_is_plain(int cfg) { return asd_gemm_tiles[cfg].kind == ASD_TILE_PLAIN; }
static bool asd_cfg_is_pp(int cfg) { return asd_gemm_tiles[cfg].kind == ASD_TILE_PP; }
static bool asd_cfg_is_ws(int cfg) { return asd_gemm_tiles[cfg].kind == ASD_TILE_WS; }
static bool asd_cfg_is_window(int cfg) { return !asd_cfg_is_plain(cfg) && !asd_cfg_is_ws(cfg); }
static int asd_cfg_wave_n(int cfg) { return asd_gemm_tiles[cfg].bn / asd_gemm_tiles[cfg].wn; }
static bool asd_conv_ws_ok(const asd_gemm_args* a) {
    return a->conv && a->stride == 1 && a->pad == 1 && a->upsample == 0 && a->Hin == 8 && a->Win == 8 && a->Hout == 8 && a->Wout == 8 &&
           a->M % 64 == 0 && a->M / 64 <= 5 && a->N % 64 == 0 && a->split_k >= 2 && a->Cin % (32 * a->split_k) == 0 && !a->gn_bwd_x && !a->ln_mode;
}

static bool asd_conv_window_ok(const asd_gemm_args* a) {
    return a->conv && a->stride == 1 && a->pad == 1 && a->upsample == 0 && a->Cin % 64 == 0 && a->Hin == a->Hout &&
           a->Win == a->Wout && a->Hout % 16 == 0 && a->Wout % 16 == 0;
}

// ... 116 lines not shown
}

int asd_gemm_plan_set(int32_t M, int32_t N, int32_t K, int32_t conv, int32_t s0, int32_t s1, int32_t s2, int32_t s3, int32_t s4,
                      int32_t tile_cfg, int32_t split_k) {
    ASD_CHECK_ARG(tile_cfg >= 0 && tile_cfg <= ASD_GEMM_NCFG && split_k >= 1, "bad plan");
    asd_plan_key k;
    memset(&k, 0, sizeof(k));
    k.M = M; k.N = N; k.K = K; k.conv = conv ? 1 : 0; k.a = s0; k.b = s1; k.c = s2; k.d = s3; k.e = s4;
    std::lock_guard<std::mutex> lk(g_plans_mu);
    g_plans[k] = asd_plan_val{tile_cfg, split_k};
    ++g_plan_gen;
    return ASD_OK;
}

int asd_gemm_plan_get(const asd_gemm_args* a, int32_t* tile_cfg, int32_t* split_k) {
    ASD_CHECK_ARG(a && tile_cfg && split_k, "null argument");
    asd_plan_val v;
    if (asd_plan_lookup(a, &v)) { *tile_cfg = v.tile; *split_k = v.split; return ASD_OK; }
    *tile_cfg = 0;
    *split_k = asd_default_split(a);
    return 1;
}

int32_t asd_gemm_gn_records(const asd_gemm_args* a_in) {
    if (!a_in || a_in->M <= 0 || a_in->N <= 0 || a_in->K <= 0) return 0;
    asd_gemm_args a = *a_in;
    asd_gemm_resolve_plan(&a);
    return asd_gemm_gn_records_cfg(&a, asd_gemm_resolve_cfg(&a), false);
}

int32_t asd_gemm_gn_applies(const asd_gemm_args* a_in) {
    if (!a_in || a_in->M <= 0 || a_in->N <= 0 || a_in->K <= 0) return 0;
    asd_gemm_args a = *a_in;
    asd_gemm_resolve_plan(&a);
    return asd_gemm_gn_apply_nv(&a) > 0 ? 1 : 0;
}

int asd_gemm_plan_count(void) {
    std::lock_guard<std::mutex> lk(g_plans_mu);
    return (int)g_plans.size();
}

int64_t asd_gemm_workspace_bytes(const asd_gemm_args* a_in) {
    if (!a_in) return 0;
    asd_gemm_args a = *a_in;
    if (a.split_k < 0) a.split_k = 0;
    asd_gemm_resolve_plan(&a);
    return a.split_k > 1 ? (int64_t)a.split_k * a.M * a.N * 4 : 0;
}

int asd_gemm_f16(const asd_gemm_args* a_in, void* stream) {
    ASD_CHECK_ARG(a_in, "null argument");
    asd_gemm_args a_copy = *a_in;
    asd_gemm_args* a = &a_copy;
    if (a->ld_row_bias <= 0) a->ld_row_bias = a->N;
    asd_gemm_resolve_plan(a);
    ASD_CHECK_ARG(a && a->A && a->W && a->C && a->zero_page, "null argument");
    ASD_CHECK_ARG(a->M > 0 && a->N > 0 && a->K > 0, "empty problem");
    ASD_CHECK_ARG(a->K % 8 == 0, "K must be a multiple of 8");
    ASD_CHECK_ARG(a->N % 4 == 0 && a->ldc % 4 == 0, "N and ldc must be multiples of 4");
    ASD_CHECK_ARG(a->ldw % 8 == 0 && (a->conv || a->lda % 8 == 0), "leading dimensions must be multiples of 8 halfs (16 B)");
    if (a->conv) {
        ASD_CHECK_ARG(a->Cin % 8 == 0 && a->K == (a->upsample == 3 ? 4 : 9) * a->Cin, "conv: Cin must be a multiple of 8 and K = 9*Cin (4*Cin in the parity form)");
        ASD_CHECK_ARG(a->upsample != 3 || (a->stride == 1 && a->Hout == 2 * a->Hin && a->Wout == 2 * a->Win && !a->gn_bwd_x),
                      "parity-form upsample conv: stride 1, Hout = 2*Hin, Wout = 2*Win");
        ASD_CHECK_ARG(a->Hout > 0 && a->Wout > 0 && a->M % (a->Hout * a->Wout) == 0, "conv: M must be B*Hout*Wout");
    }
    ASD_CHECK_ARG(a->split_k >= 1 && (a->split_k == 1 || a->workspace), "split-K needs a workspace");
    if (a->a_seg_rows > 0 || a->w_seg_rows > 0 || a->partials_only)
        ASD_CHECK_ARG(!a->conv && a->K % 64 == 0 && a->a_seg_rows >= 0 && a->w_seg_rows >= 0 && (!a->partials_only || a->split_k > 1) &&
                      (a->a_seg_rows == 0 || (a->M + a->a_seg_rows - 1) / a->a_seg_rows <= 9) && (a->w_seg_rows == 0 || (a->N + a->w_seg_rows - 1) / a->w_seg_rows <= 6),
                      "segmented rows / partials_only: plain GEMM, K % 64 == 0, at most 9 (A) and 6 (W) segments, split_k > 1 for partials_only");
    ASD_CHECK_ARG((size_t)a->N * a->ldw * 2 < ((size_t)1 << 32) && (a->conv || (size_t)a->M * a->lda * 2 < ((size_t)1 << 32)),
                  "row-major operands are addressed with 32-bit byte offsets (< 4 GiB each)");
    if (a->act == 2)
        ASD_CHECK_ARG(a->N % 32 == 0 && a->bias && !a->conv && !a->residual && !a->row_bias && !a->out_f32 && a->split_k == 1,
                      "GEGLU epilogue: N % 32 == 0, bias required, no conv / residual / row_bias / fp32 output / split-K");
    if (a->ln_mode) {
        ASD_CHECK_ARG((a->ln_mode == 1 || a->ln_mode == 2) && a->ln_sc && !a->out_f32, "LayerNorm fold: ln_mode 1 | 2, ln_sc required, fp16 output");
        ASD_CHECK_ARG(a->ln_mode == 1 || (a->ln_stats && a->N % 4 == 0), "LayerNorm fold, mode 2: the column statistics ln_stats[N][2] are required");
        ASD_CHECK_ARG(a->ln_mode == 2 || !a->conv, "LayerNorm fold, mode 1: plain GEMM only (the rows of A are the LayerNorm's rows)");
        if (a->split_k > 1) { a->split_k = 1; a->tile_cfg = 0; }
    }
    int cfg = asd_gemm_resolve_cfg(a);
    ASD_CHECK_ARG(a->act != 2 || (!asd_cfg_is_window(cfg) && asd_cfg_wave_n(cfg) % 32 == 0),
                  "GEGLU epilogue needs a tile whose per-wave width is a multiple of 32 columns");
    ASD_CHECK_ARG(asd_gemm_tiles[cfg].bn == 64 || a->N % asd_gemm_tiles[cfg].bn == 0 || (asd_gemm_tiles[cfg].bn == 128 && a->N % 4 == 0),
                  "tile configuration does not divide N");
    if (asd_gemm_gn_records_cfg(a, cfg, true) == 0) a->gn_partials = nullptr;
    {
        auto al16 = [](const void* q) { return ((uintptr_t)q & 15) == 0; };
        const int wave_n = asd_cfg_wave_n(cfg);
        a->wide_rows = wave_n % 32 == 0 && a->act != 2 && a->N % 8 == 0 && a->ldc % 8 == 0 && al16(a->C) && (!a->bias || al16(a->bias)) &&
                       (!a->row_bias || (al16(a->row_bias) && a->ld_row_bias % 8 == 0)) && (!a->residual || (al16(a->residual) && a->ldr % 8 == 0)) &&
                       !(a->gn_partials && a->gn_bwd_x);
    }
    static const bool trace = getenv("ASD_GEMM_TRACE") != nullptr;
    if (trace)
        fprintf(stderr, "ASD_GEMM %d %d %d conv=%d %d %d %d %d %d s=%d p=%d u=%d cfg=%d split=%d act=%d res=%d f32=%d gn=%d\n", a->M, a->N, a->K, a->conv, a->Hin,
                a->Win, a->Cin, a->Hout, a->Wout, a->stride, a->pad, a->upsample, cfg, a->split_k, a->act, a->residual != nullptr, a->out_f32,
                a->gn_partials ? (a->gn_bwd_x ? 2 : 1) : 0);
    if (asd_cfg_is_ws(cfg))
        ASD_CHECK_ARG(asd_conv_ws_ok(a), "weight-streaming convolution: 3x3 stride-1 pad-1 on <= 5 images of 8x8, N % 64 == 0, split_k >= 2, Cin % (32 split_k) == 0");
    if (asd_cfg_is_window(cfg)) {
        ASD_CHECK_ARG(asd_cfg_is_pp(cfg) ? asd_conv_pp_ok(a, cfg) : asd_conv_window_ok(a),
                      "window convolution needs a 3x3 stride-1 pad-1 conv with Cin % 64 == 0 (ping-pong: % 32) and H, W % 16 == 0");
        ASD_CHECK_ARG(a->split_k == 1 || a->split_k <= a->Cin / 64, "window convolution: split_k exceeds the channel chunks");
    }
    hipStream_t s = (hipStream_t)stream;
    const int rc = asd_gemm_tiles[cfg].launch(a, s);
    if (rc != ASD_OK) return rc;
    if (a->split_k > 1 && !a->partials_only) asd_launch_splitk_epilogue(a, s);
    ASD_LAUNCH_CHECK();
    return ASD_OK;
}


static int asd_tune_candidates(const asd_gemm_args* a, int (*out)[2], int max_out) {
    static const int sk_plain[] = {1, 2, 3, 4, 6, 8, 12, 16}, sk_win[] = {1, 2, 3, 4, 5, 6, 8, 10};
    const bool geglu = a->act == 2, window_ok = asd_conv_window_ok(a);
    int n = 0;
    for (int t = 0; t < ASD_GEMM_NCFG && n < max_out; ++t) {
        const int bm = asd_gemm_tiles[t].bm, bn = asd_gemm_tiles[t].bn;
        if (asd_cfg_is_ws(t)) {
            static const int sk_ws[] = {2, 4, 5, 8, 10, 16, 20};
            for (int sk : sk_ws) {
                asd_gemm_args q = *a;
                q.split_k = sk;
                if (!asd_conv_ws_ok(&q) || (a->N / 64) * sk > 512 || (a->N / 64) * sk < 64) continue;
                if (n < max_out) { out[n][0] = t + 1; out[n][1] = sk; ++n; }
            }
            continue;
        }
        if (asd_cfg_is_window(t)) {
            if (asd_cfg_is_pp(t) ? !asd_conv_pp_ok(a, t) : (!window_ok || (bn != 64 && a->N % bn != 0))) continue;
            const int tiles = (a->M / bm) * asd_div_up(a->N, bn);
            for (int sk : sk_win) {
                if (sk > 1 && (a->Cin / 64 < 2 * sk || tiles * sk > 1536)) continue;
                if (n < max_out) { out[n][0] = t + 1; out[n][1] = sk; ++n; }
            }
            continue;
        }
        if (bn != 64 && a->N % bn != 0) continue;
        const bool few = asd_gemm_tiles[t].nst > 2 || asd_gemm_tiles[t].kg > 1;
        if (few && ((a->conv && a->upsample == 2) || (long long)asd_div_up(a->M, bm) * asd_div_up(a->N, bn) > 512 || a->K < 512)) continue;
        if (geglu && asd_cfg_wave_n(t) % 32 != 0) continue;
        if (bn == 64 && a->N % 128 == 0 && a->N >= 256 && bm == 128) continue;
        const int tiles = asd_div_up(a->M, bm) * asd_div_up(a->N, bn);
        for (int sk : sk_plain) {
            if (sk > 1 && (geglu || a->K / sk < 256 || tiles * sk > 1536)) continue;
            if (few && sk != 1 && sk != 2 && sk != 4) continue;
            if (n < max_out) { out[n][0] = t + 1; out[n][1] = sk; ++n; }
        }
    }
    return n;
}

int asd_gemm_tune(const asd_gemm_args* a_in, void* scratch, int64_t scratch_bytes, void* stream) {
    ASD_CHECK_ARG(a_in, "null argument");
    hipStream_t s = (hipStream_t)stream;
    int cand[160][2];
    const int n = asd_tune_candidates(a_in, cand, 160);
    ASD_CHECK_ARG(n > 0, "no tile configuration fits this problem");
    hipEvent_t e0, e1;
    if (hipEventCreate(&e0) != hipSuccess || hipEventCreate(&e1) != hipSuccess) { asd_set_error("hipEventCreate failed"); return ASD_ERR_LAUNCH; }
    float best_ms = 1e30f;
// ... 81 lines not shown
```

### scaledreamer_amd/csrc/gemm_tile.h

```cpp
#pragma once
#include "asd_common.h"

typedef _Float16 half_t;
typedef half_t half8 __attribute__((ext_vector_type(8)));
typedef half_t half4 __attribute__((ext_vector_type(4)));
typedef float floatx4 __attribute__((ext_vector_type(4)));

enum {
    ASD_CFG_128x64 = 0, ASD_CFG_128x128 = 1, ASD_CFG_256x64 = 2, ASD_CFG_256x128 = 3, ASD_CFG_256x256 = 5, ASD_CFG_320x128 = 7,
    ASD_CFG_WIN_64 = 8, ASD_CFG_WIN_128 = 9,
    ASD_CFG_WIN2_64 = 10, ASD_CFG_WIN2_128 = 11
};

#define GLOBAL_AS __attribute__((address_space(1)))
#define LDS_AS __attribute__((address_space(3)))

__device__ __forceinline__ float gelu_erf(float x) {
    const float z = fabsf(x) * 0.70710678118654752440f;
    const float t = __builtin_amdgcn_rcpf(fmaf(0.3275911f, z, 1.f));
    float poly = fmaf(1.061405429f, t, -1.453152027f);
    poly = fmaf(poly, t, 1.421413741f);
    poly = fmaf(poly, t, -0.284496736f);
    poly = fmaf(poly, t, 0.254829592f);
    const float tail = poly * t * __builtin_amdgcn_exp2f(-1.44269504088896340736f * z * z);
// ... 21 lines not shown
__device__ __forceinline__ float row16_sum(float v) {
    int x;
#define ASD_ROW_ADD(CTRL) x = __builtin_amdgcn_update_dpp(0, __float_as_int(v), CTRL, 0xf, 0xf, true); v += __int_as_float(x)
    ASD_ROW_ADD(0x111); ASD_ROW_ADD(0x112); ASD_ROW_ADD(0x114); ASD_ROW_ADD(0x118);
#undef ASD_ROW_ADD
    return v;
}
__device__ __forceinline__ void gn_tile_begin(float* lds64) {
    __syncthreads();
    if (threadIdx.x < 64) lds64[threadIdx.x] = 0.f;
    __syncthreads();
}
__device__ __forceinline__ float silu_grad_f(float z) { return asd_silu_grad_fast(z); }
struct GnCol {
    float mean[4], rstd[4], gm[4], bt[4];
};
__device__ __forceinline__ void gn_col_load(const asd_gemm_args& p, int m_any, int n, GnCol& c) {
    if (!p.gn_bwd_x || n >= p.N) return;
    const int b = m_any / p.gn_rows;
    const float inv_cnt = 1.f / ((float)p.gn_rows * (float)p.gn_cg);
    const half4 gm = *(const half4*)((const half_t*)p.gn_bwd_gamma + n), bt = *(const half4*)((const half_t*)p.gn_bwd_beta + n);
#pragma unroll
    for (int r = 0; r < 4; ++r) {
        const int g = (n + r) / p.gn_cg;
        c.mean[r] = p.gn_bwd_fstats[(b * 32 + g) * 2] * inv_cnt;
        c.rstd[r] = rsqrtf(fmaxf(p.gn_bwd_fstats[(b * 32 + g) * 2 + 1] * inv_cnt - c.mean[r] * c.mean[r], 0.f) + p.gn_eps);
        c.gm[r] = (float)gm[r]; c.bt[r] = (float)bt[r];
    }
}
__device__ __forceinline__ void gn_tile_accum(const asd_gemm_args& p, const GnCol& c, const floatx4& o, int m, int n, floatx4& cs, floatx4& cq) {
    if (!p.gn_bwd_x) {
#pragma unroll
        for (int r = 0; r < 4; ++r) { cs[r] += o[r]; cq[r] = fmaf(o[r], o[r], cq[r]); }
        return;
    }
    const half4 xv = *(const half4*)((const half_t*)p.gn_bwd_x + (size_t)m * p.N + n);
#pragma unroll
    for (int r = 0; r < 4; ++r) {
        const float xh = ((float)xv[r] - c.mean[r]) * c.rstd[r];
        float gg = o[r] * c.gm[r];
        if (p.gn_silu) gg *= silu_grad_f(fmaf(xh, c.gm[r], c.bt[r]));
        cs[r] += gg;
        cq[r] = fmaf(gg, xh, cq[r]);
    }
}
__device__ __forceinline__ void gn_tile_flush(float* lds64, floatx4 s, floatx4 q, int n, int N, int cg) {
#pragma unroll
    for (int r = 0; r < 4; ++r) { s[r] = row16_sum(s[r]); q[r] = row16_sum(q[r]); }
    if ((threadIdx.x & 15) == 15) {
#pragma unroll
        for (int r = 0; r < 4; ++r) {
            if (n + r >= N) continue;
            const int g = (n + r) / cg;
            atomicAdd(&lds64[2 * g], s[r]);
            atomicAdd(&lds64[2 * g + 1], q[r]);
        }
    }
}
__device__ __forceinline__ void gn_tile_end(const asd_gemm_args& p, const float* lds64, int record) {
    __syncthreads();
    if (threadIdx.x < 64) p.gn_partials[(size_t)record * 64 + threadIdx.x] = lds64[threadIdx.x];
}

template <int CNT>
__device__ __forceinline__ void ln_fold(const asd_gemm_args& p, float* v, int m, int n, float mean, float rstd) {
    if (p.ln_mode == 1) {
#pragma unroll
        for (int q = 0; q < CNT / 4; ++q) {
            const floatx4 s = *(const floatx4*)(p.ln_sc + n + 4 * q), c = *(const floatx4*)(p.ln_sc + p.N + n + 4 * q);
#pragma unroll
            for (int r = 0; r < 4; ++r) v[4 * q + r] = fmaf(rstd, v[4 * q + r] - mean * s[r], c[r]);
        }
    } else {
        const float s = p.ln_sc[m], c = p.ln_sc[p.M + m];
#pragma unroll
        for (int q = 0; q < CNT / 2; ++q) {
            const floatx4 st = *(const floatx4*)(p.ln_stats + 2 * (n + 2 * q));
            v[2 * q] = fmaf(st[1], v[2 * q] - st[0] * s, c);
            v[2 * q + 1] = fmaf(st[3], v[2 * q + 1] - st[2] * s, c);
        }
    }
}

__device__ __forceinline__ floatx4 gemm_store4(const asd_gemm_args& p, floatx4 v, int m, int n) {
    if (p.bias) {
        const half4 b = *(const half4*)((const half_t*)p.bias + n);
        v[0] += (float)b[0]; v[1] += (float)b[1]; v[2] += (float)b[2]; v[3] += (float)b[3];
    }
    if (p.row_bias) {
        const half4 b = *(const half4*)((const half_t*)p.row_bias + (size_t)(m / p.rows_per_group) * p.ld_row_bias + n);
        v[0] += (float)b[0]; v[1] += (float)b[1]; v[2] += (float)b[2]; v[3] += (float)b[3];
    }
    if (p.act == 1) {
#pragma unroll
        for (int r = 0; r < 4; ++r) v[r] = asd_silu_fast(v[r]);
    }
    if (p.residual) {
        const half4 b = *(const half4*)((const half_t*)p.residual + (size_t)m * p.ldr + n);
        v[0] += (float)b[0]; v[1] += (float)b[1]; v[2] += (float)b[2]; v[3] += (float)b[3];
    }
    if (p.out_f32) {
        *(floatx4*)((float*)p.C + (size_t)m * p.ldc + n) = v;
        return v;
    }
    half4 o = {(half_t)v[0], (half_t)v[1], (half_t)v[2], (half_t)v[3]};
    *(half4*)((half_t*)p.C + (size_t)m * p.ldc + n) = o;
    return floatx4{(float)o[0], (float)o[1], (float)o[2], (float)o[3]};
}

__device__ __forceinline__ int wide_slab_rows(int ws) { return (ws >> 2) * 32 + (ws & 1) * 16 + ((ws >> 1) & 1) * 4; }
__device__ __forceinline__ int wide_lane_row(int lrow) { return (lrow >> 2) * 8 + (lrow & 3); }

__device__ __forceinline__ void gemm_store8(const asd_gemm_args& p, floatx4& lo, floatx4& hi, int m, int n) {
    float v[8] = {lo[0], lo[1], lo[2], lo[3], hi[0], hi[1], hi[2], hi[3]};
    if (p.bias) {
        const half8 b = *(const half8*)((const half_t*)p.bias + n);
#pragma unroll
        for (int k = 0; k < 8; ++k) v[k] += (float)b[k];
    }
    if (p.row_bias) {
        const half8 b = *(const half8*)((const half_t*)p.row_bias + (size_t)(m / p.rows_per_group) * p.ld_row_bias + n);
#pragma unroll
        for (int k = 0; k < 8; ++k) v[k] += (float)b[k];
    }
    if (p.act == 1) {
#pragma unroll
        for (int k = 0; k < 8; ++k) v[k] = asd_silu_fast(v[k]);
    }
    if (p.residual) {
        const half8 b = *(const half8*)((const half_t*)p.residual + (size_t)m * p.ldr + n);
#pragma unroll
        for (int k = 0; k < 8; ++k) v[k] += (float)b[k];
    }
    if (p.out_f32) {
        float* dst = (float*)p.C + (size_t)m * p.ldc + n;
        *(floatx4*)dst = floatx4{v[0], v[1], v[2], v[3]};
        *(floatx4*)(dst + 4) = floatx4{v[4], v[5], v[6], v[7]};
        lo = floatx4{v[0], v[1], v[2], v[3]}; hi = floatx4{v[4], v[5], v[6], v[7]};
        return;
    }
    const half8 o = {(half_t)v[0], (half_t)v[1], (half_t)v[2], (half_t)v[3], (half_t)v[4], (half_t)v[5], (half_t)v[6], (half_t)v[7]};
    *(half8*)((half_t*)p.C + (size_t)m * p.ldc + n) = o;
    lo = floatx4{(float)o[0], (float)o[1], (float)o[2], (float)o[3]}; hi = floatx4{(float)o[4], (float)o[5], (float)o[6], (float)o[7]};
}

template <int TM, int TN, typename RowFn>
__device__ __forceinline__ void tile_epilogue(const asd_gemm_args& p, floatx4 (&acc)[TM][TN], int nb, int kz, int row0, RowFn row, bool gn, float* gn_lds,
                                              const float* ln_mean = nullptr, const float* ln_rstd = nullptr) {
    const int g = (threadIdx.x & 63) >> 4;
    if constexpr (TN % 2 == 0) {
        if (p.wide_rows) {
#pragma unroll
            for (int s2 = 0; s2 < TN / 2; ++s2) {
                const int n = nb + s2 * 32 + g * 8;
                floatx4 cs0 = {0.f, 0.f, 0.f, 0.f}, cq0 = cs0, cs1 = cs0, cq1 = cs0;
#pragma unroll
                for (int i = 0; i < TM; ++i) {
                    const int m = row(i);
                    if (m < 0 || n >= p.N) continue;
                    if (p.split_k > 1) {
                        float* dst = p.workspace + ((size_t)kz * p.M + m) * p.N + n;
                        *(floatx4*)dst = acc[i][2 * s2];
                        *(floatx4*)(dst + 4) = acc[i][2 * s2 + 1];
                    } else {
                        floatx4 lo = acc[i][2 * s2], hi = acc[i][2 * s2 + 1];
                        if (p.ln_mode) {
                            float v8[8] = {lo[0], lo[1], lo[2], lo[3], hi[0], hi[1], hi[2], hi[3]};
                            ln_fold<8>(p, v8, m, n, ln_mean ? ln_mean[i] : 0.f, ln_rstd ? ln_rstd[i] : 0.f);
                            lo = floatx4{v8[0], v8[1], v8[2], v8[3]}; hi = floatx4{v8[4], v8[5], v8[6], v8[7]};
                        }
                        gemm_store8(p, lo, hi, m, n);
                        if (gn) {
#pragma unroll
                            for (int r = 0; r < 4; ++r) {
                                cs0[r] += lo[r]; cq0[r] = fmaf(lo[r], lo[r], cq0[r]);
                                cs1[r] += hi[r]; cq1[r] = fmaf(hi[r], hi[r], cq1[r]);
                            }
                        }
                    }
                }
                if (gn) { gn_tile_flush(gn_lds, cs0, cq0, n, p.N, p.gn_cg); gn_tile_flush(gn_lds, cs1, cq1, n + 4, p.N, p.gn_cg); }
            }
            return;
        }
    }
#pragma unroll
    for (int j = 0; j < TN; ++j) {
        const int n = nb + j * 16 + g * 4;
        floatx4 cs = {0.f, 0.f, 0.f, 0.f}, cq = {0.f, 0.f, 0.f, 0.f};
        GnCol gc;
        if (gn) gn_col_load(p, row0, n, gc);
#pragma unroll
        for (int i = 0; i < TM; ++i) {
            const int m = row(i);
            if (m < 0 || n >= p.N) continue;
            if (p.split_k > 1) *(floatx4*)(p.workspace + ((size_t)kz * p.M + m) * p.N + n) = acc[i][j];
            else {
                floatx4 a4 = acc[i][j];
                if (p.ln_mode) {
                    float v4[4] = {a4[0], a4[1], a4[2], a4[3]};
                    ln_fold<4>(p, v4, m, n, ln_mean ? ln_mean[i] : 0.f, ln_rstd ? ln_rstd[i] : 0.f);
                    a4 = floatx4{v4[0], v4[1], v4[2], v4[3]};
                }
                const floatx4 o = gemm_store4(p, a4, m, n);
                if (gn) gn_tile_accum(p, gc, o, m, n, cs, cq);
            }
        }
        if (gn) gn_tile_flush(gn_lds, cs, cq, n, p.N, p.gn_cg);
    }
}

template <int PER, int MAX>
__device__ __forceinline__ void ring_wait(int ahead) {
    if constexpr (MAX <= 0) {
        asm volatile("s_waitcnt vmcnt(0)" ::: "memory");
    } else {
        if (ahead >= MAX) asm volatile("s_waitcnt vmcnt(%0)" ::"n"(MAX * PER) : "memory");
        else ring_wait<PER, MAX - 1>(ahead);
    }
}
```

### scaledreamer_amd/csrc/net.hip

```cpp
#include <cstdlib>
#include <map>
#include <string>
#include <vector>

#include "asd_common.h"

namespace {

typedef _Float16 half_t;

struct WSpec { std::string name; int rows, cols; };

struct Bump {
    char* base = nullptr;
    size_t off = 0, cap = 0;
    void* take(size_t bytes) {
        off = (off + 255) & ~(size_t)255;
        void* p = base ? base + off : nullptr;
        off += bytes;
        return p;
    }
    half_t* halfs(size_t n) { return (half_t*)take(n * 2); }
    float* floats(size_t n) { return (float*)take(n * 4); }
};

struct Run {
    Bump mem;
    hipStream_t stream = nullptr;
    bool dry = true;
    bool tune = false;
    bool fixed = false;
    float* scratch = nullptr;
    size_t scratch_bytes = 0, scratch_need = 0;
    const void* zero_page = nullptr;
    int status = ASD_OK;
    std::vector<int>* rec_log = nullptr;
    const std::vector<int>* rec_replay = nullptr;
    size_t rec_pos = 0;
};

struct Act {
    const half_t* p = nullptr;
    const float* rec = nullptr;
    int nrec = 0;
    const half_t* applied = nullptr; const half_t* applied_gamma = nullptr; const half_t* applied_beta = nullptr;
    float applied_eps = 0.f; int applied_silu = 0;
};

struct GnNext {
    const half_t* gamma = nullptr; const half_t* beta = nullptr; float eps = 0.f; int silu = 0;
};

struct Net {
    std::vector<WSpec> specs;
    std::map<std::string, int> index;
    std::vector<const void*> ptr;
    void* zero_page = nullptr;
    bool bound = false;
    int add(const std::string& name, int rows, int cols) {
        index[name] = (int)specs.size();
        specs.push_back(WSpec{name, rows, cols});
        ptr.push_back(nullptr);
        return (int)specs.size() - 1;
    }
    const half_t* w(const std::string& name) const {
        auto it = index.find(name);
        return it == index.end() ? nullptr : (const half_t*)ptr[it->second];
    }
    bool has(const std::string& name) const { return index.count(name) != 0; }
};

int pad32(int c) { return (c + 31) / 32 * 32; }

struct GemmOpt {
    const void* bias = nullptr; const void* row_bias = nullptr; int rows_per_group = 1, ld_row_bias = 0;
    const void* residual = nullptr; int ldr = 0; int act = 0; int out_f32 = 0;
    int gn_rows = 0;
    Act* out = nullptr;
    const half_t* gn_x = nullptr; const float* gn_fstats = nullptr; const half_t* gn_gamma = nullptr; const half_t* gn_beta = nullptr;
    int gn_silu = 0;
    bool gn_bwd_form = false;
    int ln_mode = 0; const float* ln_sc = nullptr; float* ln_stats = nullptr;
    const GnNext* gn_next = nullptr;
};

void set_gn_bwd(asd_gemm_args& g, const GemmOpt& o) {
    g.gn_bwd_x = o.gn_x; g.gn_bwd_fstats = o.gn_fstats; g.gn_bwd_gamma = o.gn_gamma; g.gn_bwd_beta = o.gn_beta;
    g.gn_eps = 1e-6f; g.gn_silu = o.gn_silu;
}

void launch_gemm(Run& r, asd_gemm_args& g, Act* gn_out = nullptr, bool gn_bwd_form = false, const GnNext* gn_next = nullptr) {
    g.zero_page = r.zero_page;
    g.split_k = 0;
    g.tile_cfg = 0;
    if (r.fixed) { g.split_k = 1; g.tile_cfg = g.N % 128 == 0 ? 2 : 1; }
    if (r.tune && !r.fixed && !r.dry) {
        int32_t t, s;
        if (asd_gemm_plan_get(&g, &t, &s) != ASD_OK) {
            if (asd_gemm_tune(&g, r.scratch, (int64_t)r.scratch_bytes, r.stream) != ASD_OK) { r.status = ASD_ERR_LAUNCH; return; }
        }
    }
    const size_t need = (size_t)asd_gemm_workspace_bytes(&g);
    if (need > r.scratch_need) r.scratch_need = need;
    if (gn_bwd_form) { gn_out = nullptr; g.gn_bwd_x = nullptr; g.gn_bwd_fstats = nullptr; g.gn_bwd_gamma = nullptr; g.gn_bwd_beta = nullptr; }
    if (gn_next && gn_next->gamma && gn_out && g.gn_rows > 0 && g.N % 32 == 0 && !r.rec_replay && !r.rec_log) {
        asd_gemm_args q = g;
        q.gn_cg = g.N / 32; q.gn_apply = 1;
        const bool applies = asd_gemm_gn_applies(&q) != 0;
        half_t* y = (applies || r.tune) ? r.mem.halfs((size_t)g.M * g.N) : nullptr;
        if (applies) {
            g.gn_cg = g.N / 32; g.gn_apply = 1; g.gn_apply_y = y;
            g.gn_apply_gamma = gn_next->gamma; g.gn_apply_beta = gn_next->beta; g.gn_apply_eps = gn_next->eps; g.gn_apply_silu = gn_next->silu;
            gn_out->applied = y; gn_out->applied_gamma = gn_next->gamma; gn_out->applied_beta = gn_next->beta;
            gn_out->applied_eps = gn_next->eps; gn_out->applied_silu = gn_next->silu;
            gn_out = nullptr;
        }
    }
    if (gn_out && g.gn_rows > 0 && g.N % 32 == 0) {
        g.gn_cg = g.N / 32;
        const int batch = g.M / g.gn_rows;
        int nrec;
        if (r.rec_replay) nrec = r.rec_pos < r.rec_replay->size() ? (*r.rec_replay)[r.rec_pos++] : 0;
        else {
            asd_gemm_args q = g;
            q.gn_bwd_x = nullptr;
            nrec = asd_gemm_gn_records(&q);
        }
        const int reserve = r.tune ? (g.gn_rows / 64 + 1) * (g.N / 64 + 1) : nrec;
        if (r.rec_log) r.rec_log->push_back(nrec);
        float* buf = (nrec > 0 || r.tune) ? r.mem.floats((size_t)batch * (reserve > nrec ? reserve : nrec) * 64) : nullptr;
        if (nrec > 0) { g.gn_partials = buf; gn_out->rec = buf; gn_out->nrec = nrec; }
    }
    if (r.dry || r.status != ASD_OK) return;
    if (need > r.scratch_bytes) { asd_set_error("network workspace too small for a split-K GEMM"); r.status = ASD_ERR_ARG; return; }
    g.workspace = r.scratch;
    const int st = asd_gemm_f16(&g, r.stream);
    if (st != ASD_OK) r.status = st;
}

void gemm(Run& r, const void* A, int M, int lda, const void* W, int N, int K, int ldw, void* C, int ldc, const GemmOpt& o = GemmOpt()) {
    asd_gemm_args g = asd_gemm_args{};
    g.A = A; g.W = W; g.C = C; g.M = M; g.N = N; g.K = K; g.lda = lda; g.ldw = ldw; g.ldc = ldc;
    g.bias = o.bias; g.row_bias = o.row_bias; g.rows_per_group = o.row_bias ? o.rows_per_group : 1; g.ld_row_bias = o.ld_row_bias;
    g.residual = o.residual; g.ldr = o.ldr; g.act = o.act; g.out_f32 = o.out_f32;
    g.gn_rows = o.gn_rows;
    g.ln_mode = o.ln_mode; g.ln_sc = o.ln_sc; g.ln_stats = o.ln_stats; g.ln_eps = 1e-5f;
    if (o.gn_x) set_gn_bwd(g, o);
    if (o.out) { *o.out = Act{}; o.out->p = (const half_t*)C; }
    launch_gemm(r, g, o.out, o.gn_bwd_form, o.gn_next);
}

void conv3x3(Run& r, const void* x, int B, int Hin, int Win, int Cin, const void* W, int Cout, void* y, int Hout, int Wout, int stride,
             int pad, int upsample, const GemmOpt& o = GemmOpt()) {
    asd_gemm_args g = asd_gemm_args{};
    const int taps = upsample == 3 ? 4 : 9;
    g.A = x; g.W = W; g.C = y; g.M = B * Hout * Wout; g.N = Cout; g.K = taps * Cin; g.lda = 0; g.ldw = taps * Cin; g.ldc = Cout;
    g.bias = o.bias; g.row_bias = o.row_bias; g.rows_per_group = o.row_bias ? o.rows_per_group : 1; g.ld_row_bias = o.ld_row_bias;
    g.residual = o.residual; g.ldr = o.ldr; g.act = o.act; g.out_f32 = o.out_f32;
    g.conv = 1; g.Hin = Hin; g.Win = Win; g.Cin = Cin; g.Hout = Hout; g.Wout = Wout; g.stride = stride; g.pad = pad; g.upsample = upsample;
    g.gn_rows = o.gn_rows;
    if (o.gn_x) set_gn_bwd(g, o);
    if (o.out) { *o.out = Act{}; o.out->p = (const half_t*)y; }
    launch_gemm(r, g, o.out, o.gn_bwd_form, o.gn_next);
}

#define LEAF(call)                                              \
    do {                                                        \
        if (!r.dry && r.status == ASD_OK) {                     \
            const int st__ = (call);                            \
            if (st__ != ASD_OK) r.status = st__;                \
        }                                                       \
    } while (0)

half_t* groupnorm(Run& r, const void* x1, int c1, const void* x2, int c2, int B, int hw, const half_t* gamma, const half_t* beta, float eps,
                  int silu, half_t* y = nullptr, float** stats_out = nullptr, const Act* src = nullptr) {
    if (src && src->applied && !x2 && !y && !stats_out && src->applied_gamma == gamma && src->applied_beta == beta && src->applied_eps == eps &&
        src->applied_silu == silu)
        return const_cast<half_t*>(src->applied);
    if (!y) y = r.mem.halfs((size_t)B * hw * (c1 + c2));
    float* stats = r.mem.floats(ASD_GN_STATS_FLOATS(B));
    if (src && src->nrec > 0 && !x2) {
        LEAF(asd_groupnorm_apply_f16(x1, c1, B, hw, gamma, beta, eps, silu, src->rec, src->nrec, y, stats, r.stream));
    } else
    LEAF(asd_groupnorm_f16(x1, c1, x2, c2, B, hw, gamma, beta, eps, silu, y, stats, r.stream));
    if (stats_out) *stats_out = stats;
    return y;
}

struct ULayer { int kind; std::string name; int cin, cout; };
struct UBlock { std::vector<ULayer> layers; };

struct UNet : Net {
    asd_unet_desc d;
    std::vector<UBlock> inputs, outputs;
    UBlock middle;
    std::map<std::string, int> emb_off, ctx_off;
    int emb_total = 0, ctx_total = 0;
};

#define ASD_LN_FOLD_MIN_C 1024
void u_norm(UNet& n, const std::string& p, int c) { n.add(p + ".weight", 1, c); n.add(p + ".bias", 1, c); }
void u_lin(UNet& n, const std::string& p, int cin, int cout, bool bias = true) { n.add(p + ".weight", cout, cin); if (bias) n.add(p + ".bias", 1, cout); }
void u_conv(UNet& n, const std::string& p, int cin, int cout) { n.add(p + ".weight", cout, 9 * pad32(cin)); n.add(p + ".bias", 1, cout); }

void u_res(UNet& n, const std::string& p, int cin, int cout) {
    u_norm(n, p + ".in_layers.0", cin);
    u_conv(n, p + ".in_layers.2", cin, cout);
    u_norm(n, p + ".out_layers.0", cout);
    u_conv(n, p + ".out_layers.3", cout, cout);
    if (cin != cout) u_lin(n, p + ".skip_connection", cin, cout);
    n.emb_off[p] = n.emb_total;
    n.emb_total += cout;
}
void u_attn(UNet& n, const std::string& p, int c) {
    u_norm(n, p + ".norm", c);
    u_lin(n, p + ".proj_in", c, c);
    for (int dd = 0; dd < n.d.transformer_depth; ++dd) {
        const std::string b = p + ".transformer_blocks." + std::to_string(dd);
        const bool fold = c >= ASD_LN_FOLD_MIN_C;
        if (!fold) for (const char* nm : {".norm1", ".norm2", ".norm3"}) u_norm(n, b + nm, c);
        n.add(b + ".attn1.to_qk.weight", 2 * c, c);
        if (fold) n.add(b + ".attn1.to_qk.ln_sc", 1, 4 * 2 * c);
        n.add(b + ".attn1.to_v.weight", c, c);
        if (fold) n.add(b + ".attn1.to_v.ln_sc", 1, 4 * c);
        u_lin(n, b + ".attn1.to_out.0", c, c);
        n.add(b + ".attn2.to_q.weight", c, c);
        if (fold) n.add(b + ".attn2.to_q.ln_sc", 1, 4 * c);
        u_lin(n, b + ".attn2.to_out.0", c, c);
        u_lin(n, b + ".ff.net.0.proj", c, 8 * c);
// ... 42 lines not shown
    for (int lvl = d.n_levels - 1; lvl >= 0; --lvl) {
        const int mult = d.channel_mult[lvl];
        for (int i = 0; i <= d.num_res_blocks; ++i) {
            const int ich = chans.back();
            chans.pop_back();
            const std::string p = "output_blocks." + std::to_string(n.outputs.size());
            UBlock b;
            u_res(n, p + ".0", ch + ich, mc * mult);
            b.layers.push_back(ULayer{1, p + ".0", ch + ich, mc * mult});
            ch = mc * mult;
            int k = 1;
            if (d.attention_ds_mask & (1 << ds)) {
                u_attn(n, p + "." + std::to_string(k), ch);
                b.layers.push_back(ULayer{2, p + "." + std::to_string(k), ch, ch});
                ++k;
            }
            if (lvl && i == d.num_res_blocks) {
                const std::string q = p + "." + std::to_string(k) + ".conv";
                n.add(q + ".weight", 4 * ch, 4 * pad32(ch)); n.add(q + ".bias", 1, ch);
                b.layers.push_back(ULayer{4, q, ch, ch});
                --ds;
            }
            n.outputs.push_back(b);
        }
    }
    u_norm(n, "out.0", ch);
    u_conv(n, "out.2", mc, d.out_channels);
    n.add("emb_all.weight", n.emb_total, emb);
    n.add("emb_all.bias", 1, n.emb_total);
    n.add("ctx_k_all.weight", n.ctx_total, d.context_dim);
    n.add("ctx_v_all.weight", n.ctx_total, d.context_dim);
}

struct UState {
    int B, F, n_ctx, ctx_stride;
    const half_t* emb_all; int emb_ld;
    const half_t* k_all; const half_t* vT_all;
    const UState* full = nullptr;
    const int* expand = nullptr;
};

half_t* gather_rows(Run& r, const half_t* src, const int* idx, int n_out, size_t row_halfs) {
    half_t* dst = r.mem.halfs((size_t)n_out * row_halfs);
    LEAF(asd_gather_rows_f16(src, idx, n_out, (int64_t)row_halfs, dst, r.stream));
    return dst;
}

Act u_resblock(UNet& n, Run& r, const UState& s, const std::string& p, const Act& xin, int cin, int cout, int Hh, int Ww, const GnNext* next = nullptr) {
    const int B = s.B, hw = Hh * Ww, M = B * hw;
    const half_t* x = xin.p;
    half_t* t1 = groupnorm(r, x, cin, nullptr, 0, B, hw, n.w(p + ".in_layers.0.weight"), n.w(p + ".in_layers.0.bias"), 1e-5f, 1, nullptr, nullptr, &xin);
    half_t* t2 = r.mem.halfs((size_t)M * cout);
    Act a2;
    GemmOpt o1;
    o1.bias = n.w(p + ".in_layers.2.bias");
    o1.row_bias = s.emb_all + n.emb_off[p]; o1.rows_per_group = hw; o1.ld_row_bias = s.emb_ld;
    o1.gn_rows = hw; o1.out = &a2;
    const GnNext gn2{n.w(p + ".out_layers.0.weight"), n.w(p + ".out_layers.0.bias"), 1e-5f, 1};
    o1.gn_next = &gn2;
    conv3x3(r, t1, B, Hh, Ww, cin, n.w(p + ".in_layers.2.weight"), cout, t2, Hh, Ww, 1, 1, 0, o1);
    half_t* t3 = groupnorm(r, t2, cout, nullptr, 0, B, hw, n.w(p + ".out_layers.0.weight"), n.w(p + ".out_layers.0.bias"), 1e-5f, 1, nullptr, nullptr, &a2);
    const half_t* skip = x;
    if (n.has(p + ".skip_connection.weight")) {
        half_t* sk = r.mem.halfs((size_t)M * cout);
        GemmOpt os;
        os.bias = n.w(p + ".skip_connection.bias");
        gemm(r, x, M, cin, n.w(p + ".skip_connection.weight"), cout, cin, cin, sk, cout, os);
        skip = sk;
    }
    half_t* out = r.mem.halfs((size_t)M * cout);
    Act ao;
    GemmOpt o2;
    o2.bias = n.w(p + ".out_layers.3.bias"); o2.residual = skip; o2.ldr = cout; o2.gn_rows = hw; o2.out = &ao; o2.gn_next = next;
    conv3x3(r, t3, B, Hh, Ww, cout, n.w(p + ".out_layers.3.weight"), cout, out, Hh, Ww, 1, 1, 0, o2);
    return ao;
}

half_t* layernorm(Run& r, const half_t* x, int rows, int c, const half_t* g, const half_t* b) {
    half_t* y = r.mem.halfs((size_t)rows * c);
    LEAF(asd_layernorm_f16(x, rows, c, g, b, 1e-5f, y, r.stream));
    return y;
}

Act u_transformer(UNet& n, Run& r, const UState& s_in, const std::string& p, const Act& xin, int C, int Hh, int Ww, const GnNext* next = nullptr) {
    const UState* sp = &s_in;
    int B = sp->B, L = Hh * Ww, M = B * L;
    const int heads = C / 64, F = sp->F;
    const half_t* x = xin.p;
    half_t* h = groupnorm(r, x, C, nullptr, 0, B, L, n.w(p + ".norm.weight"), n.w(p + ".norm.bias"), 1e-6f, 0, nullptr, nullptr, &xin);
    {
        half_t* h2 = r.mem.halfs((size_t)M * C);
        GemmOpt o; o.bias = n.w(p + ".proj_in.bias");
        gemm(r, h, M, C, n.w(p + ".proj_in.weight"), C, C, C, h2, C, o);
        h = h2;
    }
    for (int dd = 0; dd < n.d.transformer_depth; ++dd) {
        const std::string b = p + ".transformer_blocks." + std::to_string(dd);
        const bool fold = n.has(b + ".attn1.to_qk.ln_sc");
        GemmOpt oqk, ov;
        const half_t* y = h;
        if (fold) {
            float* lnst = r.mem.floats((size_t)M * 2);
            oqk.ln_mode = 1; oqk.ln_sc = (const float*)n.w(b + ".attn1.to_qk.ln_sc"); oqk.ln_stats = lnst;
            ov.ln_mode = 2; ov.ln_sc = (const float*)n.w(b + ".attn1.to_v.ln_sc"); ov.ln_stats = lnst;
        } else y = layernorm(r, h, M, C, n.w(b + ".norm1.weight"), n.w(b + ".norm1.bias"));
        half_t* qk = r.mem.halfs((size_t)M * 2 * C);
        gemm(r, y, M, C, n.w(b + ".attn1.to_qk.weight"), 2 * C, C, C, qk, 2 * C, oqk);
        half_t* vT = r.mem.halfs((size_t)C * M);
        gemm(r, n.w(b + ".attn1.to_v.weight"), C, C, y, M, C, C, vT, M, ov);
        half_t* o1 = r.mem.halfs((size_t)M * C);
        LEAF(asd_attention_f16(qk, 2 * C, qk + C, 2 * C, vT, M, o1, C, B / F, heads, F * L, F * L, F * L, 0.125f, r.zero_page, r.stream));
        half_t* h1 = r.mem.halfs((size_t)M * C);
        { GemmOpt o; o.bias = n.w(b + ".attn1.to_out.0.bias"); o.residual = h; o.ldr = C;
          gemm(r, o1, M, C, n.w(b + ".attn1.to_out.0.weight"), C, C, C, h1, C, o); }
        if (sp->full) {
            const UState* f = sp->full;
            h1 = gather_rows(r, h1, sp->expand, f->B, (size_t)L * C);
            x = gather_rows(r, x, sp->expand, f->B, (size_t)L * C);
            sp = f; B = f->B; M = B * L;
        }
        const UState& s = *sp;
        half_t* q = r.mem.halfs((size_t)M * C);
        { GemmOpt o;
          y = h1;
          if (fold) { o.ln_mode = 1; o.ln_sc = (const float*)n.w(b + ".attn2.to_q.ln_sc"); }
          else y = layernorm(r, h1, M, C, n.w(b + ".norm2.weight"), n.w(b + ".norm2.bias"));
          gemm(r, y, M, C, n.w(b + ".attn2.to_q.weight"), C, C, C, q, C, o); }
        const int coff = n.ctx_off[b + ".attn2"], ldv = B * s.ctx_stride;
        half_t* o2 = r.mem.halfs((size_t)M * C);
        LEAF(asd_attention_f16(q, C, s.k_all + coff, n.ctx_total, s.vT_all + (size_t)coff * ldv, ldv, o2, C, B, heads, L, s.n_ctx, s.ctx_stride,
                               0.125f, r.zero_page, r.stream));
        half_t* h2 = r.mem.halfs((size_t)M * C);
        { GemmOpt o; o.bias = n.w(b + ".attn2.to_out.0.bias"); o.residual = h1; o.ldr = C;
          gemm(r, o2, M, C, n.w(b + ".attn2.to_out.0.weight"), C, C, C, h2, C, o); }
        half_t* g = r.mem.halfs((size_t)M * 4 * C);
        { GemmOpt o; o.bias = n.w(b + ".ff.net.0.proj.bias"); o.act = 2;
          y = h2;
          if (fold) { o.ln_mode = 1; o.ln_sc = (const float*)n.w(b + ".ff.net.0.proj.ln_sc"); }
          else y = layernorm(r, h2, M, C, n.w(b + ".norm3.weight"), n.w(b + ".norm3.bias"));
          gemm(r, y, M, C, n.w(b + ".ff.net.0.proj.weight"), 8 * C, C, C, g, 4 * C, o); }
        half_t* h3 = r.mem.halfs((size_t)M * C);
        { GemmOpt o; o.bias = n.w(b + ".ff.net.2.bias"); o.residual = h2; o.ldr = C;
          gemm(r, g, M, 4 * C, n.w(b + ".ff.net.2.weight"), C, 4 * C, 4 * C, h3, C, o); }
        h = h3;
    }
    half_t* out = r.mem.halfs((size_t)M * C);
    Act ao;
    GemmOpt o; o.bias = n.w(p + ".proj_out.bias"); o.residual = x; o.ldr = C; o.gn_rows = L; o.out = &ao; o.gn_next = next;
    gemm(r, h, M, C, n.w(p + ".proj_out.weight"), C, C, C, out, C, o);
    return ao;
}

bool u_first_norm(UNet& n, const ULayer* l, GnNext* out) {
    if (!l) return false;
    if (l->kind == 1) { *out = GnNext{n.w(l->name + ".in_layers.0.weight"), n.w(l->name + ".in_layers.0.bias"), 1e-5f, 1}; return true; }
    if (l->kind == 2) { *out = GnNext{n.w(l->name + ".norm.weight"), n.w(l->name + ".norm.bias"), 1e-6f, 0}; return true; }
    return false;
}

Act u_apply(UNet& n, Run& r, const UState& s, const UBlock& blk, Act h, int* Hh, int* Ww, const ULayer* after = nullptr) {
    for (size_t li = 0; li < blk.layers.size(); ++li) {
        const ULayer& l = blk.layers[li];
        const int B = s.B;
        GnNext gnn;
        const GnNext* next = u_first_norm(n, li + 1 < blk.layers.size() ? &blk.layers[li + 1] : after, &gnn) ? &gnn : nullptr;
        if (l.kind == 0) {
            half_t* y = r.mem.halfs((size_t)B * *Hh * *Ww * l.cout);
            Act a;
            GemmOpt o; o.bias = n.w(l.name + ".bias"); o.gn_rows = *Hh * *Ww; o.out = &a;
            conv3x3(r, h.p, B, *Hh, *Ww, pad32(l.cin), n.w(l.name + ".weight"), l.cout, y, *Hh, *Ww, 1, 1, 0, o);
            h = a;
        } else if (l.kind == 1) {
            h = u_resblock(n, r, s, l.name, h, l.cin, l.cout, *Hh, *Ww, next);
        } else if (l.kind == 2) {
            h = u_transformer(n, r, s, l.name, h, l.cout, *Hh, *Ww, next);
        } else if (l.kind == 3) {
            const int Ho = (*Hh + 2 - 3) / 2 + 1, Wo = (*Ww + 2 - 3) / 2 + 1;
            half_t* y = r.mem.halfs((size_t)B * Ho * Wo * l.cout);
            Act a;
            GemmOpt o; o.bias = n.w(l.name + ".bias"); o.gn_rows = Ho * Wo; o.out = &a; o.gn_next = next;
            conv3x3(r, h.p, B, *Hh, *Ww, l.cin, n.w(l.name + ".weight"), l.cout, y, Ho, Wo, 2, 1, 0, o);
            h = a; *Hh = Ho; *Ww = Wo;
        } else {
            half_t* y = r.mem.halfs((size_t)B * 4 * *Hh * *Ww * l.cout);
            Act a;
            GemmOpt o; o.bias = n.w(l.name + ".bias"); o.gn_rows = 4 * *Hh * *Ww; o.out = &a;
            conv3x3(r, h.p, B, *Hh, *Ww, l.cin, n.w(l.name + ".weight"), l.cout, y, 2 * *Hh, 2 * *Ww, 1, 1, 3, o);
            h = a; *Hh *= 2; *Ww *= 2;
        }
    }
    return h;
}

void unet_run(UNet& n, Run& r, const half_t* x, const float* t, const half_t* ctx, const half_t* camera, int B, int Hh, int Ww, int n_ctx,
// ... 756 lines not shown
```

### scaledreamer_amd/diffusion/hip_ops.py

```python
from __future__ import annotations

import ctypes as C
import os
from typing import Optional

import torch

from .. import _lib as L
from .._lib import GemmArgs, check, f32, i32, lib, ptr, stream

_zero = {}
_gn_stats = {}


def zero_page(device) -> torch.Tensor:
    key = str(device)
    if key not in _zero:
        _zero[key] = torch.zeros(256, dtype=torch.uint8, device=device)
    return _zero[key]


def _p(t: Optional[torch.Tensor]):
    return None if t is None else C.c_void_p(t.data_ptr())

# ... 11 lines not shown

KIND_PLAIN, KIND_WIN, KIND_WIN2, KIND_PP, KIND_WS = range(5)
TILES = tile_table()
TILE_BM = tuple(r[1] for r in TILES)
TILE_BN = tuple(r[2] for r in TILES)
WINDOW_TILES = tuple(i for i, r in enumerate(TILES) if r[0] in (KIND_WIN, KIND_WIN2, KIND_PP))
PP_TILES = tuple(i for i, r in enumerate(TILES) if r[0] == KIND_PP)
WS_TILE = next((i for i, r in enumerate(TILES) if r[0] == KIND_WS), None)
AUTOTUNE = os.environ.get("ASD_GEMM_AUTOTUNE", "1") != "0"
PLAN_FILE = os.environ.get("ASD_GEMM_PLAN_FILE", os.path.join(os.path.dirname(os.path.abspath(__file__)), "gemm_plans.json"))
TUNE_SCRATCH_BYTES = 512 << 20
_tune_scratch = {}


def _sig(key):
    M, N, K, tail = key
    if isinstance(tail, tuple):
        return (M, N, K, 1) + tuple(int(v) for v in tail)
    return (M, N, K, 0, int(tail), 0, 0, 0, 0)


def load_plans(path: str = PLAN_FILE) -> int:
    import ast
    import json

    if not os.path.exists(path):
        return 0
    with open(path) as f:
        table = json.load(f)
    for k, v in table.items():
        check(lib().asd_gemm_plan_set(*[i32(x) for x in _sig(ast.literal_eval(k))], i32(int(v[0])), i32(int(v[1]))))
    return len(table)


def plan_table() -> dict:
    out = {}
    buf = (C.c_int32 * 11)()
    for i in range(lib().asd_gemm_plan_count()):
        check(lib().asd_gemm_plan_entry(i32(i), buf))
        M, N, K, conv, s0, s1, s2, s3, s4, tile, sk = list(buf)
        out[(M, N, K, (s0, s1, s2, s3, s4) if conv else s0)] = (tile, sk)
    return out


def save_plans(path: str = PLAN_FILE) -> None:
    import json

    with open(path, "w") as f:
        json.dump({repr(k): list(v) for k, v in sorted(plan_table().items(), key=lambda kv: repr(kv[0]))}, f, indent=0)


def plan_of(g: GemmArgs):
    t, sk = C.c_int32(0), C.c_int32(1)
    tuned = lib().asd_gemm_plan_get(C.byref(g), C.byref(t), C.byref(sk)) == 0
    return (t.value, sk.value) if tuned else None


def default_split(M: int, N: int, K: int) -> int:
    g = GemmArgs()
    g.M, g.N, g.K, g.lda = M, N, K, K
    t, sk = C.c_int32(0), C.c_int32(1)
    lib().asd_gemm_plan_get(C.byref(g), C.byref(t), C.byref(sk))
    return sk.value


def tune_scratch(device) -> torch.Tensor:
    key = str(device)
    if key not in _tune_scratch:
        _tune_scratch[key] = torch.empty(TUNE_SCRATCH_BYTES, dtype=torch.uint8, device=device)
    return _tune_scratch[key]


def release_tune_scratch() -> None:
    _tune_scratch.clear()


if os.environ.get("ASD_GEMM_PLAN_FILE", "") != "none" and os.path.exists(L.LIB_PATH):
    load_plans()


def gemm(a: torch.Tensor, w: torch.Tensor, bias=None, row_bias=None, rows_per_group: int = 0, residual=None, act: int = 0,
         out: Optional[torch.Tensor] = None, out_f32: bool = False, split_k: Optional[int] = None, conv: Optional[dict] = None,
         M: Optional[int] = None, tile_cfg: int = 0, gn_rows: int = 0, gn_bwd: Optional[dict] = None, ln: Optional[dict] = None,
         gn_apply: Optional[dict] = None):
    dev = a.device
    N, K = w.shape
    if conv is not None and int(conv.get("upsample", 0)) == 3:
        N //= 4
    if conv is None:
        assert a.stride(-1) == 1 and a.dim() == 2
        M = a.shape[0]
        lda = a.stride(0)
    else:
        lda = 0
    if out is None:
        out = torch.empty((M, N // 2 if act == 2 else N), device=dev, dtype=torch.float32 if out_f32 else torch.float16)
    g = GemmArgs()
    g.A, g.W, g.C = a.data_ptr(), w.data_ptr(), out.data_ptr()
    g.M, g.N, g.K = M, N, K
    g.lda, g.ldw, g.ldc = lda, w.stride(0), out.stride(0)
    g.bias = None if bias is None else bias.data_ptr()
    g.row_bias = None if row_bias is None else row_bias.data_ptr()
    if row_bias is not None:
        assert row_bias.stride(-1) == 1 and row_bias.shape[-1] == N, "row_bias: [groups, N] with unit column stride"
        g.ld_row_bias = row_bias.stride(0) if row_bias.dim() == 2 and row_bias.shape[0] > 1 else N
    g.rows_per_group = rows_per_group if row_bias is not None else 1
    g.residual = None if residual is None else residual.data_ptr()
    g.ldr = 0 if residual is None else residual.stride(0)
    g.act, g.out_f32 = act, int(out_f32)
    if conv is not None:
        g.conv = 1
        for k in ("Hin", "Win", "Cin", "Hout", "Wout", "stride", "pad", "upsample"):
            setattr(g, k, int(conv[k]))
    g.zero_page = zero_page(dev).data_ptr()
    g.tile_cfg = tile_cfg
    if ln is not None:
        g.ln_mode, g.ln_eps, g.ln_sc = int(ln["mode"]), float(ln.get("eps", 1e-5)), ln["sc"].data_ptr()
        g.ln_stats = None if ln.get("stats") is None else ln["stats"].data_ptr()
    if split_k is not None:
        g.split_k = split_k
    else:
        g.split_k = 0
        if AUTOTUNE and plan_of(g) is None and not torch.cuda.is_current_stream_capturing():
            sc = tune_scratch(dev)
            check(lib().asd_gemm_tune(C.byref(g), C.c_void_p(sc.data_ptr()), C.c_int64(sc.numel()), stream()))
    need = lib().asd_gemm_workspace_bytes(C.byref(g))
    ws = None
    if need > 0:
        ws = torch.empty(need, device=dev, dtype=torch.uint8)
        g.workspace = ws.data_ptr()
    rec, nrec = None, 0
    if gn_rows > 0 and gn_apply is not None:
        g.gn_cg, g.gn_rows, g.gn_apply = N // 32, gn_rows, 1
        y = st = None
        if lib().asd_gemm_gn_applies(C.byref(g)):
            y = torch.empty((M, N), device=dev, dtype=torch.float16)
            st = torch.empty((M // gn_rows, 64), device=dev, dtype=torch.float32)
            g.gn_apply_y, g.gn_apply_stats = y.data_ptr(), st.data_ptr()
            g.gn_apply_gamma, g.gn_apply_beta = gn_apply["gamma"].data_ptr(), gn_apply["beta"].data_ptr()
            g.gn_apply_eps, g.gn_apply_silu = float(gn_apply["eps"]), int(gn_apply["silu"])
        check(lib().asd_gemm_f16(C.byref(g), stream()))
        return out, y, st
    if gn_rows > 0:
        g.gn_cg, g.gn_rows = N // 32, gn_rows
        if gn_bwd is not None:
            g.gn_bwd_x, g.gn_bwd_fstats = gn_bwd["x"].data_ptr(), gn_bwd["fstats"].data_ptr()
            g.gn_bwd_gamma, g.gn_bwd_beta = gn_bwd["gamma"].data_ptr(), gn_bwd["beta"].data_ptr()
            g.gn_eps, g.gn_silu = float(gn_bwd["eps"]), int(gn_bwd["silu"])
        nrec = lib().asd_gemm_gn_records(C.byref(g))
        if nrec > 0:
            rec = torch.empty((M // gn_rows, nrec, 64), device=dev, dtype=torch.float32)
            g.gn_partials = rec.data_ptr()
    check(lib().asd_gemm_f16(C.byref(g), stream()))
    return (out, rec, nrec) if gn_rows > 0 else out


def conv3x3(x: torch.Tensor, w_packed: torch.Tensor, bias=None, stride: int = 1, pad: int = 1, upsample: bool = False,
            out_hw=None, **kw) -> torch.Tensor:
    B, H, W_, Cin = x.shape
    assert x.is_contiguous()
    if out_hw is None:
        if upsample == 2:
            raise ValueError("transposed-conv mode needs out_hw")
        if upsample:
            Ho, Wo = 2 * H, 2 * W_
        else:
            Ho, Wo = (H + 2 * pad - 3) // stride + 1, (W_ + 2 * pad - 3) // stride + 1
    else:
        Ho, Wo = out_hw
    conv = dict(Hin=H, Win=W_, Cin=Cin, Hout=Ho, Wout=Wo, stride=stride, pad=pad, upsample=int(upsample))
    y = gemm(x, w_packed, bias=bias, conv=conv, M=B * Ho * Wo, **kw)
    cout = w_packed.shape[0] // 4 if int(upsample) == 3 else w_packed.shape[0]
    if isinstance(y, tuple):
        return y[0].view(B, Ho, Wo, cout), y[1], y[2]
    return y.view(B, Ho, Wo, cout)


def pack_upsample_conv3x3_weight(w: torch.Tensor) -> torch.Tensor:
    from .weights import _pack_upsample_conv3x3

    return _pack_upsample_conv3x3(w).contiguous()


def pack_conv3x3_weight(w: torch.Tensor, cin_pad: Optional[int] = None) -> torch.Tensor:
    from .weights import _pack_conv3x3

    return _pack_conv3x3(w, cin_pad).contiguous()


def groupnorm(x1: torch.Tensor, gamma, beta, eps: float, silu: bool, x2: Optional[torch.Tensor] = None,
              return_stats: bool = False):
    B = x1.shape[0]
    c1 = x1.shape[-1]
    c2 = 0 if x2 is None else x2.shape[-1]
    hw = x1.numel() // (B * c1)
    y = torch.empty(tuple(x1.shape[:-1]) + (c1 + c2,), device=x1.device, dtype=torch.float16)
    stats = torch.empty(B * 64 + (512 + B) * 64, device=x1.device, dtype=torch.float32)
    check(lib().asd_groupnorm_f16(ptr(x1), i32(c1), _p(x2), i32(c2), i32(B), i32(hw), ptr(gamma), ptr(beta), f32(eps),
# ... 27 lines not shown
def groupnorm_bwd_apply(x: torch.Tensor, dy: torch.Tensor, gamma, beta, eps: float, silu: bool, stats: torch.Tensor, records: torch.Tensor,
                        dx_add: Optional[torch.Tensor] = None) -> torch.Tensor:
    B, c = x.shape[0], x.shape[-1]
    hw = x.numel() // (B * c)
    dx = torch.empty_like(x)
    bstats = torch.empty((512 + B) * 64, device=x.device, dtype=torch.float32)
    check(lib().asd_groupnorm_bwd_apply_f16(ptr(x), ptr(dy), i32(c), i32(B), i32(hw), ptr(gamma), ptr(beta), f32(eps), i32(int(silu)),
                                            ptr(stats), ptr(records), i32(records.shape[1]), ptr(dx_add), ptr(dx), ptr(bstats), stream()))
    return dx


def transpose(x: torch.Tensor) -> torch.Tensor:
    rows, cols = x.shape
    y = torch.empty((cols, rows), device=x.device, dtype=torch.float16)
    check(lib().asd_transpose_f16(C.c_void_p(x.data_ptr()), i32(rows), i32(cols), i32(x.stride(0)), ptr(y), i32(rows), stream()))
    return y


def softmax(x: torch.Tensor, scale: float = 1.0) -> torch.Tensor:
    rows, cols = x.shape
    y = torch.empty((rows, cols), device=x.device, dtype=torch.float16)
    check(lib().asd_softmax_f16(C.c_void_p(x.data_ptr()), i32(x.stride(0)), i32(rows), i32(cols), f32(scale), ptr(y), i32(cols), stream()))
    return y


def softmax_bwd(p: torch.Tensor, dp: torch.Tensor, scale: float = 1.0) -> torch.Tensor:
    rows, cols = p.shape
    assert p.is_contiguous() and dp.is_contiguous()
    ds = torch.empty_like(p)
    check(lib().asd_softmax_bwd_f16(ptr(p), ptr(dp), i32(cols), i32(rows), i32(cols), f32(scale), ptr(ds), stream()))
    return ds


def layernorm(x: torch.Tensor, gamma, beta, eps: float = 1e-5) -> torch.Tensor:
    c = x.shape[-1]
    y = torch.empty_like(x)
    check(lib().asd_layernorm_f16(ptr(x), i32(x.numel() // c), i32(c), ptr(gamma), ptr(beta), f32(eps), ptr(y), stream()))
    return y


def pack_geglu_weight(w: torch.Tensor, b: torch.Tensor):
    from .weights import _geglu_rows

    perm = _geglu_rows(w.shape[0] // 2).to(w.device)
    return w[perm].contiguous(), b[perm].contiguous()


def geglu(h: torch.Tensor) -> torch.Tensor:
    c = h.shape[-1] // 2
    y = torch.empty(tuple(h.shape[:-1]) + (c,), device=h.device, dtype=torch.float16)
    check(lib().asd_geglu_f16(ptr(h), i32(h.numel() // (2 * c)), i32(c), ptr(y), stream()))
    return y


def silu(x: torch.Tensor) -> torch.Tensor:
    y = torch.empty_like(x)
    check(lib().asd_silu_f16(ptr(x), C.c_int64(x.numel()), ptr(y), stream()))
    return y


def timestep_embedding(t: torch.Tensor, dim: int) -> torch.Tensor:
    t = t.float().contiguous()
    y = torch.empty((t.shape[0], dim), device=t.device, dtype=torch.float16)
    check(lib().asd_timestep_embedding_f16(ptr(t), i32(t.shape[0]), i32(dim), ptr(y), stream()))
    return y


def concat(x1: torch.Tensor, x2: torch.Tensor) -> torch.Tensor:
    c1, c2 = x1.shape[-1], x2.shape[-1]
    y = torch.empty(tuple(x1.shape[:-1]) + (c1 + c2,), device=x1.device, dtype=torch.float16)
    check(lib().asd_concat_f16(ptr(x1), i32(c1), ptr(x2), i32(c2), C.c_int64(x1.numel() // c1), ptr(y), stream()))
    return y


def attention(q: torch.Tensor, k: torch.Tensor, vT: torch.Tensor, batch: int, heads: int, lq: int, lk: int,
              lk_stride: Optional[int] = None, scale: Optional[float] = None) -> torch.Tensor:
    lk_stride = lk if lk_stride is None else lk_stride
    o = torch.empty((batch * lq, heads * 64), device=q.device, dtype=torch.float16)
    check(lib().asd_attention_f16(C.c_void_p(q.data_ptr()), i32(q.stride(0)), C.c_void_p(k.data_ptr()), i32(k.stride(0)),
                                  C.c_void_p(vT.data_ptr()), i32(vT.stride(0)), ptr(o), i32(o.stride(0)), i32(batch), i32(heads),
                                  i32(lq), i32(lk), i32(lk_stride), f32(scale if scale is not None else 64 ** -0.5),
                                  ptr(zero_page(q.device)), stream()))
    return o
```

Before: 73.74 steps/s.

## Fold softmax scale into Q projection and add single-pass short-key attention

Adds an output-scale epilogue to the GEMM so the Q projection is pre-multiplied by the softmax scale times log2(e). A log2-domain attention kernel variant (MODE 1) then skips the per-score FMA and seeds the score accumulator with the running max, rescaling only when a wave's max grows past a threshold. A separate MODE 2 path handles key lengths of 80 or fewer (the cross-attention case) in one pass with no online-softmax rescaling. The cost is extra template instantiations, and f16 Q values now carry the scale, which can change rounding slightly.

```diff
diff --git a/include/asd_hip.h b/include/asd_hip.h
--- a/include/asd_hip.h
+++ b/include/asd_hip.h
@@ -290,6 +290,8 @@
     float   gn_apply_eps;
     int32_t gn_apply_silu;
     float*  gn_apply_stats;
+    float   out_scale;
+    int32_t out_scale_cols;
 } asd_gemm_args;
 int32_t asd_gemm_gn_records(const asd_gemm_args* args);
 int32_t asd_gemm_gn_applies(const asd_gemm_args* args);
@@ -327,6 +329,9 @@
 int asd_attention_f16(const void* q, int32_t ldq, const void* k, int32_t ldk, const void* vT, int32_t ldv,
                       void* o, int32_t ldo, int32_t batch, int32_t heads, int32_t lq, int32_t lk,
                       int32_t lk_stride, float scale, const void* zero_page, void* stream);
+int asd_attention_log2_f16(const void* q, int32_t ldq, const void* k, int32_t ldk, const void* vT, int32_t ldv,
+                           void* o, int32_t ldo, int32_t batch, int32_t heads, int32_t lq, int32_t lk,
+                           int32_t lk_stride, const void* zero_page, void* stream);
 
 int asd_gemm_plan_set(int32_t M, int32_t N, int32_t K, int32_t conv, int32_t s0, int32_t s1, int32_t s2, int32_t s3, int32_t s4,
                       int32_t tile_cfg, int32_t split_k);
diff --git a/scaledreamer_amd/_lib.py b/scaledreamer_amd/_lib.py
--- a/scaledreamer_amd/_lib.py
+++ b/scaledreamer_amd/_lib.py
@@ -80,6 +80,7 @@
         ("partials_only", C.c_int32),
         ("gn_apply", C.c_int32), ("gn_apply_y", C.c_void_p), ("gn_apply_gamma", C.c_void_p), ("gn_apply_beta", C.c_void_p),
         ("gn_apply_eps", C.c_float), ("gn_apply_silu", C.c_int32), ("gn_apply_stats", C.c_void_p),
+        ("out_scale", C.c_float), ("out_scale_cols", C.c_int32),
     ]
 
 
@@ -163,7 +164,7 @@
     "asd_generate_rays", "asd_march_count", "asd_scan_i32", "asd_march_write", "asd_prune_count", "asd_compact",
     "asd_occgrid_update", "asd_composite_fwd", "asd_composite_bwd",
     "asd_gemm_f16", "asd_gemm_force_tile", "asd_groupnorm_f16", "asd_groupnorm_bwd_f16", "asd_transpose_f16", "asd_layernorm_f16", "asd_softmax_f16", "asd_softmax_bwd_f16", "asd_geglu_f16", "asd_silu_f16",
-    "asd_timestep_embedding_f16", "asd_concat_f16", "asd_attention_f16",
+    "asd_timestep_embedding_f16", "asd_concat_f16", "asd_attention_f16", "asd_attention_log2_f16",
     "asd_gemm_plan_set", "asd_gemm_plan_get", "asd_gemm_plan_count", "asd_gemm_plan_generation", "asd_gemm_plan_entry", "asd_gemm_tile_info", "asd_gemm_workspace_bytes", "asd_gemm_tune", "asd_gemm_gn_records", "asd_gemm_gn_applies", "asd_groupnorm_apply_f16", "asd_groupnorm_bwd_apply_f16", "asd_groupnorm_ordered_f16",
     "asd_pad_cast_f16",
     "asd_image_prep_fwd", "asd_image_prep_bwd", "asd_latents_fwd", "asd_score_fwd", "asd_latents_bwd", "asd_prompt_context",
diff --git a/scaledreamer_amd/csrc/attention.hip b/scaledreamer_amd/csrc/attention.hip
--- a/scaledreamer_amd/csrc/attention.hip
+++ b/scaledreamer_amd/csrc/attention.hip
@@ -24,6 +24,18 @@
     v = max3f(__uint_as_float(t[0]), __uint_as_float(t[1]), -3.0e38f);
     t = __builtin_amdgcn_permlane32_swap(__float_as_uint(v), __float_as_uint(v), false, false);
     return max3f(__uint_as_float(t[0]), __uint_as_float(t[1]), -3.0e38f);
+}
+
+__device__ __forceinline__ float max2f(float a, float b) {
+    float r;
+    asm("v_max_f32 %0, %1, %2" : "=v"(r) : "v"(a), "v"(b));
+    return r;
+}
+__device__ __forceinline__ float rows_max2(float v) {
+    auto t = __builtin_amdgcn_permlane16_swap(__float_as_uint(v), __float_as_uint(v), false, false);
+    v = max2f(__uint_as_float(t[0]), __uint_as_float(t[1]));
+    t = __builtin_amdgcn_permlane32_swap(__float_as_uint(v), __float_as_uint(v), false, false);
+    return max2f(__uint_as_float(t[0]), __uint_as_float(t[1]));
 }
 
 #define HD 64
@@ -40,7 +52,7 @@
     const char* zero;
 };
 
-template <int QS>
+template <int QS, int MODE>
 __global__ __launch_bounds__(256, QS == 2 ? 4 : 2) void attention_fwd_kernel(const AttnArgs p) {
     constexpr int QW = 16 * QS, QB = 4 * QW;
     extern __shared__ __attribute__((aligned(16))) char smem[];
@@ -101,8 +113,97 @@
     const half_t one_or_zero = lq16 == 0 ? (half_t)1.f : (half_t)0.f;
     const half8 ones_row0 = {one_or_zero, one_or_zero, one_or_zero, one_or_zero, one_or_zero, one_or_zero, one_or_zero, one_or_zero};
 
+    const float sl2 = p.scale * 1.44269504088896340736f;
+    if constexpr (MODE == 2) {
+        issue(0, 0);
+        issue(1, 1);
+        __builtin_amdgcn_s_waitcnt(0);
+        __syncthreads();
+        const char* K0 = smem;
+        const char* V0 = smem + TILE_BYTES;
+        const char* K1 = smem + 2 * TILE_BYTES;
+        const char* V1 = smem + 3 * TILE_BYTES;
+        floatx4 s[5][QS];
+#pragma unroll
+        for (int kt = 0; kt < 5; ++kt) {
+            const int row = (kt & 3) * 16 + lq16;
+            const char* Ks = kt < 4 ? K0 : K1;
+            half8 kf[2];
+#pragma unroll
+            for (int ks = 0; ks < 2; ++ks) kf[ks] = *(const half8*)(Ks + row * 128 + (((ks * 4 + lg) ^ (row & 7)) * 16));
+#pragma unroll
+            for (int qs = 0; qs < QS; ++qs) {
+                floatx4 a = {0.f, 0.f, 0.f, 0.f};
+                a = __builtin_amdgcn_mfma_f32_16x16x32_f16(kf[0], qf[qs][0], a, 0, 0, 0);
+                a = __builtin_amdgcn_mfma_f32_16x16x32_f16(kf[1], qf[qs][1], a, 0, 0, 0);
+                s[kt][qs] = a;
+            }
+        }
+        if (p.lk < 80) {
+#pragma unroll
+            for (int qs = 0; qs < QS; ++qs)
+#pragma unroll
+                for (int kt = 0; kt < 5; ++kt)
+#pragma unroll
+                    for (int r = 0; r < 4; ++r)
+                        if (kt * 16 + lg * 4 + r >= p.lk) s[kt][qs][r] = -1e30f;
+        }
+        half8 pb[2][QS];
+        half4 pt[QS];
+#pragma unroll
+        for (int qs = 0; qs < QS; ++qs) {
+            const float a0 = max3f(s[0][qs][0], s[0][qs][1], s[0][qs][2]), a1 = max3f(s[0][qs][3], s[1][qs][0], s[1][qs][1]);
+            const float a2 = max3f(s[1][qs][2], s[1][qs][3], s[2][qs][0]), a3 = max3f(s[2][qs][1], s[2][qs][2], s[2][qs][3]);
+            const float a4 = max3f(s[3][qs][0], s[3][qs][1], s[3][qs][2]), a5 = max3f(s[4][qs][0], s[4][qs][1], s[4][qs][2]);
+            float mx = max3f(max3f(a0, a1, a2), max3f(a3, a4, s[3][qs][3]), max2f(a5, s[4][qs][3]));
+            mx = rows_max2(mx);
+            const float nm = -mx * sl2;
+#pragma unroll
+            for (int kt = 0; kt < 5; ++kt) {
+                const float e0 = __builtin_amdgcn_exp2f(__builtin_fmaf(s[kt][qs][0], sl2, nm)), e1 = __builtin_amdgcn_exp2f(__builtin_fmaf(s[kt][qs][1], sl2, nm));
+                const float e2 = __builtin_amdgcn_exp2f(__builtin_fmaf(s[kt][qs][2], sl2, nm)), e3 = __builtin_amdgcn_exp2f(__builtin_fmaf(s[kt][qs][3], sl2, nm));
+                if (kt < 4) {
+                    half8& dst = pb[kt >> 1][qs];
+                    dst[(kt & 1) * 4 + 0] = (half_t)e0; dst[(kt & 1) * 4 + 1] = (half_t)e1;
+                    dst[(kt & 1) * 4 + 2] = (half_t)e2; dst[(kt & 1) * 4 + 3] = (half_t)e3;
+                } else pt[qs] = half4{(half_t)e0, (half_t)e1, (half_t)e2, (half_t)e3};
+            }
+        }
+#pragma unroll
+        for (int j = 0; j < 2; ++j) {
+#pragma unroll
+            for (int dt = 0; dt < 4; ++dt) {
+                const int row = dt * 16 + lq16;
+                const int sw = (row >> 1) & 7;
+                const int c_lo = (4 * j + (lg >> 1)) ^ sw, c_hi = (4 * j + 2 + (lg >> 1)) ^ sw;
+                const half4 v_lo = *(const volatile LDS_AS half4*)(V0 + row * 128 + c_lo * 16 + (lg & 1) * 8);
+                const half4 v_hi = *(const volatile LDS_AS half4*)(V0 + row * 128 + c_hi * 16 + (lg & 1) * 8);
+                const half8 vf = half8{v_lo[0], v_lo[1], v_lo[2], v_lo[3], v_hi[0], v_hi[1], v_hi[2], v_hi[3]};
+#pragma unroll
+                for (int qs = 0; qs < QS; ++qs) oacc[qs][dt] = __builtin_amdgcn_mfma_f32_16x16x32_f16(vf, pb[j][qs], oacc[qs][dt], 0, 0, 0);
+            }
+#pragma unroll
+            for (int qs = 0; qs < QS; ++qs) lacc[qs] = __builtin_amdgcn_mfma_f32_16x16x32_f16(ones_row0, pb[j][qs], lacc[qs], 0, 0, 0);
+        }
+        {
+            const half4 ones4 = {one_or_zero, one_or_zero, one_or_zero, one_or_zero};
+#pragma unroll
+            for (int dt = 0; dt < 4; ++dt) {
+                const int row = dt * 16 + lq16;
+                const int c = (lg >> 1) ^ ((row >> 1) & 7);
+                const half4 vf = *(const volatile LDS_AS half4*)(V1 + row * 128 + c * 16 + (lg & 1) * 8);
+#pragma unroll
+                for (int qs = 0; qs < QS; ++qs) oacc[qs][dt] = __builtin_amdgcn_mfma_f32_16x16x16f16(vf, pt[qs], oacc[qs][dt], 0, 0, 0);
+            }
+#pragma unroll
+            for (int qs = 0; qs < QS; ++qs) lacc[qs] = __builtin_amdgcn_mfma_f32_16x16x16f16(ones4, pt[qs], lacc[qs], 0, 0, 0);
+        }
+    } else {
     const int n_tiles = (p.lk + KT - 1) / KT;
-    const float sl2 = p.scale * 1.44269504088896340736f;
+    if constexpr (MODE == 1) {
+#pragma unroll
+        for (int qs = 0; qs < QS; ++qs) m_run[qs] = 0.f;
+    }
     issue(0, 0);
     __builtin_amdgcn_s_waitcnt(0);
     __syncthreads();
@@ -122,6 +223,7 @@
 #pragma unroll
             for (int qs = 0; qs < QS; ++qs) {
                 floatx4 a = {0.f, 0.f, 0.f, 0.f};
+                if constexpr (MODE == 1) a = floatx4{m_run[qs], m_run[qs], m_run[qs], m_run[qs]};
                 a = __builtin_amdgcn_mfma_f32_16x16x32_f16(kf[0], qf[qs][0], a, 0, 0, 0);
                 a = __builtin_amdgcn_mfma_f32_16x16x32_f16(kf[1], qf[qs][1], a, 0, 0, 0);
                 s[kt][qs] = a;
@@ -144,8 +246,34 @@
             const float a0 = max3f(s[0][qs][0], s[0][qs][1], s[0][qs][2]), a1 = max3f(s[0][qs][3], s[1][qs][0], s[1][qs][1]);
             const float a2 = max3f(s[1][qs][2], s[1][qs][3], s[2][qs][0]), a3 = max3f(s[2][qs][1], s[2][qs][2], s[2][qs][3]);
             const float a4 = max3f(s[3][qs][0], s[3][qs][1], s[3][qs][2]);
-            float mx = max3f(max3f(a0, a1, a2), max3f(a3, a4, s[3][qs][3]), -3.0e38f);
-            mx = rows_max(mx);
+            float mx;
+            if constexpr (MODE == 1) mx = rows_max2(max2f(max3f(a0, a1, a2), max3f(a3, a4, s[3][qs][3])));
+            else mx = rows_max(max3f(max3f(a0, a1, a2), max3f(a3, a4, s[3][qs][3]), -3.0e38f));
+            if constexpr (MODE == 1) {
+                const bool grow = t == 0 || __builtin_amdgcn_ballot_w64(mx > ATTN_DEFER_LOG2) != 0;
+                if (grow) {
+                    const float m_old = t == 0 ? -3.0e38f : -m_run[qs];
+                    const float m_new = max2f(m_old, mx - m_run[qs]);
+                    const float alpha = __builtin_amdgcn_exp2f(m_old - m_new), d = m_new + m_run[qs];
+#pragma unroll
+                    for (int kt = 0; kt < 4; ++kt) { s[kt][qs][0] -= d; s[kt][qs][1] -= d; s[kt][qs][2] -= d; s[kt][qs][3] -= d; }
+#pragma unroll
+                    for (int dt = 0; dt < 4; ++dt) {
+                        oacc[qs][dt][0] *= alpha; oacc[qs][dt][1] *= alpha; oacc[qs][dt][2] *= alpha; oacc[qs][dt][3] *= alpha;
+                    }
+                    lacc[qs][0] *= alpha;
+                    m_run[qs] = -m_new;
+                }
+#pragma unroll
+                for (int kt = 0; kt < 4; ++kt) {
+                    const float e0 = __builtin_amdgcn_exp2f(s[kt][qs][0]), e1 = __builtin_amdgcn_exp2f(s[kt][qs][1]);
+                    const float e2 = __builtin_amdgcn_exp2f(s[kt][qs][2]), e3 = __builtin_amdgcn_exp2f(s[kt][qs][3]);
+                    half8& dst = pb[kt >> 1][qs];
+                    dst[(kt & 1) * 4 + 0] = (half_t)e0; dst[(kt & 1) * 4 + 1] = (half_t)e1;
+                    dst[(kt & 1) * 4 + 2] = (half_t)e2; dst[(kt & 1) * 4 + 3] = (half_t)e3;
+                }
+                continue;
+            }
             const float cand = mx * sl2;
             const bool grow = __builtin_amdgcn_ballot_w64(cand > m_run[qs] + ATTN_DEFER_LOG2) != 0;
             const float m_new = grow ? max3f(m_run[qs], cand, -3.0e38f) : m_run[qs];
@@ -194,6 +322,7 @@
         }
         __syncthreads();
     }
+    }
 
 #pragma unroll
     for (int qs = 0; qs < QS; ++qs) {
@@ -224,13 +353,37 @@
     const bool wide = lk >= 2048 && lq >= 2048;
     if (wide) {
         const dim3 grid(8 * asd_div_up(asd_div_up(lq, 256) * heads * batch, 8));
-        hipLaunchKernelGGL(attention_fwd_kernel<4>, grid, dim3(256), 4 * KT * HD * 2, (hipStream_t)stream, a);
+        hipLaunchKernelGGL((attention_fwd_kernel<4, 0>), grid, dim3(256), 4 * KT * HD * 2, (hipStream_t)stream, a);
     } else {
         const dim3 grid(8 * asd_div_up(asd_div_up(lq, 128) * heads * batch, 8));
-        hipLaunchKernelGGL(attention_fwd_kernel<2>, grid, dim3(256), 4 * KT * HD * 2, (hipStream_t)stream, a);
+        if (lk <= 80) hipLaunchKernelGGL((attention_fwd_kernel<2, 2>), grid, dim3(256), 4 * KT * HD * 2, (hipStream_t)stream, a);
+        else hipLaunchKernelGGL((attention_fwd_kernel<2, 0>), grid, dim3(256), 4 * KT * HD * 2, (hipStream_t)stream, a);
     }
     ASD_LAUNCH_CHECK();
     return ASD_OK;
 }
 
-}
+int asd_attention_log2_f16(const void* q, int32_t ldq, const void* k, int32_t ldk, const void* vT, int32_t ldv, void* o,
+                           int32_t ldo, int32_t batch, int32_t heads, int32_t lq, int32_t lk, int32_t lk_stride,
+                           const void* zero_page, void* stream) {
+    ASD_CHECK_ARG(q && k && vT && o && zero_page, "null argument");
+    ASD_CHECK_ARG(batch > 0 && heads > 0 && lq > 0 && lk > 0 && lk_stride >= lk, "bad sizes");
+    ASD_CHECK_ARG(ldq % 8 == 0 && ldk % 8 == 0 && ldv % 8 == 0 && ldo % 4 == 0 && lk_stride % 8 == 0,
+                  "leading dimensions / key stride must keep 16-byte alignment");
+    AttnArgs a{(const half_t*)q, ldq, (const half_t*)k, ldk, (const half_t*)vT, ldv, (half_t*)o, ldo,
+               batch, heads, lq, lk, lk_stride, 0.69314718055994530942f , (const char*)zero_page};
+    if (lk >= 2048 && lq >= 2048) {
+        const dim3 grid(8 * asd_div_up(asd_div_up(lq, 256) * heads * batch, 8));
+        hipLaunchKernelGGL((attention_fwd_kernel<4, 1>), grid, dim3(256), 4 * KT * HD * 2, (hipStream_t)stream, a);
+    } else {
+        const dim3 grid(8 * asd_div_up(asd_div_up(lq, 128) * heads * batch, 8));
+        if (lk <= 80) hipLaunchKernelGGL((attention_fwd_kernel<2, 2>), grid, dim3(256), 4 * KT * HD * 2, (hipStream_t)stream, a);
+        else {
+            hipLaunchKernelGGL((attention_fwd_kernel<2, 0>), grid, dim3(256), 4 * KT * HD * 2, (hipStream_t)stream, a);
+        }
+    }
+    ASD_LAUNCH_CHECK();
+    return ASD_OK;
+}
+
+}
diff --git a/scaledreamer_amd/csrc/gemm.hip b/scaledreamer_amd/csrc/gemm.hip
--- a/scaledreamer_amd/csrc/gemm.hip
+++ b/scaledreamer_amd/csrc/gemm.hip
@@ -10,7 +10,7 @@
 #include "gemm_tile.h"
 
 
-template <int BM, int BN, int WM, int WN, bool CONV, int NST = 2, int KG = 1, bool LN = false>
+template <int BM, int BN, int WM, int WN, bool CONV, int NST = 2, int KG = 1, bool LN = false, bool OSC = false>
 __global__ __launch_bounds__(WM * WN * KG * 64) void gemm_f16_kernel(const asd_gemm_args p) {
     constexpr int NW = WM * WN;
     constexpr int TM = BM / WM / 16, TN = BN / WN / 16;
@@ -386,7 +386,7 @@
     const bool gn = p.gn_partials != nullptr;
     float* gn_lds = (float*)smem;
     if (gn) gn_tile_begin(gn_lds);
-    tile_epilogue<TM, TN>(p, acc, n0 + wn * (BN / WN), kz, m0, out_row, gn, gn_lds, LN ? ln_mean : nullptr, LN ? ln_rstd : nullptr);
+    tile_epilogue<TM, TN, OSC>(p, acc, n0 + wn * (BN / WN), kz, m0, out_row, gn, gn_lds, LN ? ln_mean : nullptr, LN ? ln_rstd : nullptr);
     if (gn) gn_tile_end(p, gn_lds, (m0 / BM) * ((p.N + BN - 1) / BN) + n0 / BN);
 }
 
@@ -692,6 +692,9 @@
         const half4 b = *(const half4*)((const half_t*)p.row_bias + (size_t)(m / p.rows_per_group) * p.ld_row_bias + n);
         v[0] += (float)b[0]; v[1] += (float)b[1]; v[2] += (float)b[2]; v[3] += (float)b[3];
     }
+    if (n < p.out_scale_cols) {
+        v[0] *= p.out_scale; v[1] *= p.out_scale; v[2] *= p.out_scale; v[3] *= p.out_scale;
+    }
     if (p.act == 1) {
 #pragma unroll
         for (int r = 0; r < 4; ++r) v[r] = asd_silu_fast(v[r]);
@@ -909,6 +912,8 @@
     if (a->group_m < 1 || a->group_n < 1) asd_pick_group(asd_div_up(a->M, BM), asd_div_up(a->N, BN), BM, BN, lds, &a->group_m, &a->group_n);
     const dim3 grid(8 * asd_div_up(tiles * a->split_k, 8)), block(WM * WN * KG * 64);
     if (a->conv) asd_launch_lds<gemm_f16_kernel<BM, BN, WM, WN, true, NST, KG, false>>(grid, block, lds, s, *a);
+    else if (a->out_scale_cols != 0 && a->ln_mode == 1) asd_launch_lds<gemm_f16_kernel<BM, BN, WM, WN, false, NST, KG, true, true>>(grid, block, lds, s, *a);
+    else if (a->out_scale_cols != 0) asd_launch_lds<gemm_f16_kernel<BM, BN, WM, WN, false, NST, KG, false, true>>(grid, block, lds, s, *a);
     else if (a->ln_mode == 1) asd_launch_lds<gemm_f16_kernel<BM, BN, WM, WN, false, NST, KG, true>>(grid, block, lds, s, *a);
     else asd_launch_lds<gemm_f16_kernel<BM, BN, WM, WN, false, NST, KG, false>>(grid, block, lds, s, *a);
     return ASD_OK;
@@ -1191,6 +1196,10 @@
         ASD_CHECK_ARG(a->ln_mode == 2 || !a->conv, "LayerNorm fold, mode 1: plain GEMM only (the rows of A are the LayerNorm's rows)");
         if (a->split_k > 1) { a->split_k = 1; a->tile_cfg = 0; }
     }
+    if (a->out_scale_cols != 0)
+        ASD_CHECK_ARG(a->out_scale_cols > 0 && a->out_scale_cols % 8 == 0 && a->out_scale_cols <= a->N && a->act != 2 && !a->out_f32 && !a->conv &&
+                      !a->partials_only && !a->gn_partials && !a->gn_apply,
+                      "out_scale: a multiple of 8 columns <= N; not with GEGLU, fp32 output, convolutions, partials_only or GroupNorm epilogues");
     int cfg = asd_gemm_resolve_cfg(a);
     ASD_CHECK_ARG(a->act != 2 || (!asd_cfg_is_window(cfg) && asd_cfg_wave_n(cfg) % 32 == 0),
                   "GEGLU epilogue needs a tile whose per-wave width is a multiple of 32 columns");
diff --git a/scaledreamer_amd/csrc/gemm_tile.h b/scaledreamer_amd/csrc/gemm_tile.h
--- a/scaledreamer_amd/csrc/gemm_tile.h
+++ b/scaledreamer_amd/csrc/gemm_tile.h
@@ -127,6 +127,7 @@
     }
 }
 
+template <bool SCALED = false>
 __device__ __forceinline__ floatx4 gemm_store4(const asd_gemm_args& p, floatx4 v, int m, int n) {
     if (p.bias) {
         const half4 b = *(const half4*)((const half_t*)p.bias + n);
@@ -136,6 +137,10 @@
         const half4 b = *(const half4*)((const half_t*)p.row_bias + (size_t)(m / p.rows_per_group) * p.ld_row_bias + n);
         v[0] += (float)b[0]; v[1] += (float)b[1]; v[2] += (float)b[2]; v[3] += (float)b[3];
     }
+    if constexpr (SCALED) {
+        const float f = n < p.out_scale_cols ? p.out_scale : 1.f;
+        v[0] *= f; v[1] *= f; v[2] *= f; v[3] *= f;
+    }
     if (p.act == 1) {
 #pragma unroll
         for (int r = 0; r < 4; ++r) v[r] = asd_silu_fast(v[r]);
@@ -156,6 +161,7 @@
 __device__ __forceinline__ int wide_slab_rows(int ws) { return (ws >> 2) * 32 + (ws & 1) * 16 + ((ws >> 1) & 1) * 4; }
 __device__ __forceinline__ int wide_lane_row(int lrow) { return (lrow >> 2) * 8 + (lrow & 3); }
 
+template <bool SCALED = false>
 __device__ __forceinline__ void gemm_store8(const asd_gemm_args& p, floatx4& lo, floatx4& hi, int m, int n) {
     float v[8] = {lo[0], lo[1], lo[2], lo[3], hi[0], hi[1], hi[2], hi[3]};
     if (p.bias) {
@@ -167,6 +173,11 @@
         const half8 b = *(const half8*)((const half_t*)p.row_bias + (size_t)(m / p.rows_per_group) * p.ld_row_bias + n);
 #pragma unroll
         for (int k = 0; k < 8; ++k) v[k] += (float)b[k];
+    }
+    if constexpr (SCALED) {
+        const float f = n < p.out_scale_cols ? p.out_scale : 1.f;
+#pragma unroll
+        for (int k = 0; k < 8; ++k) v[k] *= f;
     }
     if (p.act == 1) {
 #pragma unroll
@@ -189,7 +200,7 @@
     lo = floatx4{(float)o[0], (float)o[1], (float)o[2], (float)o[3]}; hi = floatx4{(float)o[4], (float)o[5], (float)o[6], (float)o[7]};
 }
 
-template <int TM, int TN, typename RowFn>
+template <int TM, int TN, bool SCALED = false, typename RowFn>
 __device__ __forceinline__ void tile_epilogue(const asd_gemm_args& p, floatx4 (&acc)[TM][TN], int nb, int kz, int row0, RowFn row, bool gn, float* gn_lds,
                                               const float* ln_mean = nullptr, const float* ln_rstd = nullptr) {
     const int g = (threadIdx.x & 63) >> 4;
@@ -214,7 +225,7 @@
                             ln_fold<8>(p, v8, m, n, ln_mean ? ln_mean[i] : 0.f, ln_rstd ? ln_rstd[i] : 0.f);
                             lo = floatx4{v8[0], v8[1], v8[2], v8[3]}; hi = floatx4{v8[4], v8[5], v8[6], v8[7]};
                         }
-                        gemm_store8(p, lo, hi, m, n);
+                        gemm_store8<SCALED>(p, lo, hi, m, n);
                         if (gn) {
 #pragma unroll
                             for (int r = 0; r < 4; ++r) {
@@ -247,7 +258,7 @@
                     ln_fold<4>(p, v4, m, n, ln_mean ? ln_mean[i] : 0.f, ln_rstd ? ln_rstd[i] : 0.f);
                     a4 = floatx4{v4[0], v4[1], v4[2], v4[3]};
                 }
-                const floatx4 o = gemm_store4(p, a4, m, n);
+                const floatx4 o = gemm_store4<SCALED>(p, a4, m, n);
                 if (gn) gn_tile_accum(p, gc, o, m, n, cs, cq);
             }
         }
diff --git a/scaledreamer_amd/csrc/net.hip b/scaledreamer_amd/csrc/net.hip
--- a/scaledreamer_amd/csrc/net.hip
+++ b/scaledreamer_amd/csrc/net.hip
@@ -81,6 +81,7 @@
     int gn_silu = 0;
     bool gn_bwd_form = false;
     int ln_mode = 0; const float* ln_sc = nullptr; float* ln_stats = nullptr;
+    float out_scale = 0.f; int out_scale_cols = 0;
     const GnNext* gn_next = nullptr;
 };
 
@@ -145,6 +146,7 @@
     g.residual = o.residual; g.ldr = o.ldr; g.act = o.act; g.out_f32 = o.out_f32;
     g.gn_rows = o.gn_rows;
     g.ln_mode = o.ln_mode; g.ln_sc = o.ln_sc; g.ln_stats = o.ln_stats; g.ln_eps = 1e-5f;
+    g.out_scale = o.out_scale; g.out_scale_cols = o.out_scale_cols;
     if (o.gn_x) set_gn_bwd(g, o);
     if (o.out) { *o.out = Act{}; o.out->p = (const half_t*)C; }
     launch_gemm(r, g, o.out, o.gn_bwd_form, o.gn_next);
@@ -353,6 +355,8 @@
     return y;
 }
 
+static const float ATTN_Q_SCALE = 0.125f * 1.44269504088896340736f;
+
 Act u_transformer(UNet& n, Run& r, const UState& s_in, const std::string& p, const Act& xin, int C, int Hh, int Ww, const GnNext* next = nullptr) {
     const UState* sp = &s_in;
     int B = sp->B, L = Hh * Ww, M = B * L;
@@ -369,6 +373,8 @@
         const std::string b = p + ".transformer_blocks." + std::to_string(dd);
         const bool fold = n.has(b + ".attn1.to_qk.ln_sc");
         GemmOpt oqk, ov;
+        const bool log2_self = F * L >= 2048;
+        if (log2_self) { oqk.out_scale = ATTN_Q_SCALE; oqk.out_scale_cols = C; }
         const half_t* y = h;
         if (fold) {
             float* lnst = r.mem.floats((size_t)M * 2);
@@ -380,7 +386,8 @@
         half_t* vT = r.mem.halfs((size_t)C * M);
         gemm(r, n.w(b + ".attn1.to_v.weight"), C, C, y, M, C, C, vT, M, ov);
         half_t* o1 = r.mem.halfs((size_t)M * C);
-        LEAF(asd_attention_f16(qk, 2 * C, qk + C, 2 * C, vT, M, o1, C, B / F, heads, F * L, F * L, F * L, 0.125f, r.zero_page, r.stream));
+        if (log2_self) LEAF(asd_attention_log2_f16(qk, 2 * C, qk + C, 2 * C, vT, M, o1, C, B / F, heads, F * L, F * L, F * L, r.zero_page, r.stream));
+        else LEAF(asd_attention_f16(qk, 2 * C, qk + C, 2 * C, vT, M, o1, C, B / F, heads, F * L, F * L, F * L, 0.125f, r.zero_page, r.stream));
         half_t* h1 = r.mem.halfs((size_t)M * C);
         { GemmOpt o; o.bias = n.w(b + ".attn1.to_out.0.bias"); o.residual = h; o.ldr = C;
           gemm(r, o1, M, C, n.w(b + ".attn1.to_out.0.weight"), C, C, C, h1, C, o); }
diff --git a/scaledreamer_amd/diffusion/hip_ops.py b/scaledreamer_amd/diffusion/hip_ops.py
--- a/scaledreamer_amd/diffusion/hip_ops.py
+++ b/scaledreamer_amd/diffusion/hip_ops.py
@@ -117,7 +117,7 @@
 def gemm(a: torch.Tensor, w: torch.Tensor, bias=None, row_bias=None, rows_per_group: int = 0, residual=None, act: int = 0,
          out: Optional[torch.Tensor] = None, out_f32: bool = False, split_k: Optional[int] = None, conv: Optional[dict] = None,
          M: Optional[int] = None, tile_cfg: int = 0, gn_rows: int = 0, gn_bwd: Optional[dict] = None, ln: Optional[dict] = None,
-         gn_apply: Optional[dict] = None):
+         gn_apply: Optional[dict] = None, out_scale: float = 0.0, out_scale_cols: int = 0):
     dev = a.device
     N, K = w.shape
     if conv is not None and int(conv.get("upsample", 0)) == 3:
@@ -149,6 +149,7 @@
             setattr(g, k, int(conv[k]))
     g.zero_page = zero_page(dev).data_ptr()
     g.tile_cfg = tile_cfg
+    g.out_scale, g.out_scale_cols = float(out_scale), int(out_scale_cols)
     if ln is not None:
         g.ln_mode, g.ln_eps, g.ln_sc = int(ln["mode"]), float(ln.get("eps", 1e-5)), ln["sc"].data_ptr()
         g.ln_stats = None if ln.get("stats") is None else ln["stats"].data_ptr()
@@ -342,3 +343,16 @@
                                   i32(lq), i32(lk), i32(lk_stride), f32(scale if scale is not None else 64 ** -0.5),
                                   ptr(zero_page(q.device)), stream()))
     return o
+
+
+LOG2E = 1.4426950408889634
+
+
+def attention_log2(q: torch.Tensor, k: torch.Tensor, vT: torch.Tensor, batch: int, heads: int, lq: int, lk: int,
+                   lk_stride: Optional[int] = None) -> torch.Tensor:
+    lk_stride = lk if lk_stride is None else lk_stride
+    o = torch.empty((batch * lq, heads * 64), device=q.device, dtype=torch.float16)
+    check(lib().asd_attention_log2_f16(C.c_void_p(q.data_ptr()), i32(q.stride(0)), C.c_void_p(k.data_ptr()), i32(k.stride(0)),
+                                       C.c_void_p(vT.data_ptr()), i32(vT.stride(0)), ptr(o), i32(o.stride(0)), i32(batch), i32(heads),
+                                       i32(lq), i32(lk), i32(lk_stride), ptr(zero_page(q.device)), stream()))
+    return o
```

Measured after the change: 74.09 steps/s (median of 6 runs). Within noise of the previous version (+0.5%).
